# liangfu/dspnet

Hardware: AMD Instinct MI355X
Metric: training images/sec at 512x512 multitask (higher is better)
Workload: dtype f32; 1 GPU; resnet-50 multitask (det+depth+seg) 512x512, 8 det classes, 19 seg classes, N=6132 anchors, forward+backward+SGD; batch_per_gpu=32, global_batch=32, parallelism=dp1, f16x2_fallback_calls=0

## Files before the change

### dspnet_amd/csrc/conv.hip

```cpp
#include "dspn_common.h"
#include "bn_final_job.h"
#include "dspn_store.h"
#include "dspn_pieces.h"
#include "conv_geom.h"
#include <cstdlib>
#include "../../include/dspn_nn.h"

using dspn::st_t;
using dspn::kHalf;
using dspn::u32x4_t;

namespace {

using dspn::conv::f32x16;
using dspn::conv::bf16x8;
using dspn::pieces::bf16x4;
typedef __attribute__((address_space(3))) bf16x4 lds_bf16x4;

constexpr int kLdsRowH = kHalf ? 72 : 40;
__device__ __forceinline__ bf16x4 to_bf16x4(const float4 v) {
  bf16x4 r = {(__bf16)v.x, (__bf16)v.y, (__bf16)v.z, (__bf16)v.w};
  return r;
}

// ... 1227 lines not shown
  auto lo = [](int num, int den) { return num <= 0 ? 0 : (num + den - 1) / den; };
  const int ho_lo = lo(g.ph - r * g.dh, g.sh), wo_lo = lo(g.pw - q * g.dw, g.sw);
  const int ho_hi = min(g.Ho - 1, (g.H - 1 + g.ph - r * g.dh) / g.sh);
  const int wo_hi = min(g.Wo - 1, (g.W - 1 + g.pw - q * g.dw) / g.sw);
  const int rows_per = (g.Ho + g.chunks - 1) / g.chunks;
  const int h0 = max(ho_lo, chunk * rows_per), h1 = min(ho_hi, (chunk + 1) * rows_per - 1);
  const int KL = min(g.ldy, 256), PL = 256 / KL;
  const int kl = threadIdx.x % KL, pl = threadIdx.x / KL;
  for (int kb = 0; kb < g.ldy; kb += KL) {
    const int k = kb + kl;
    float s = 0.f;
    if (pl < PL && k < g.ldy && (g.H - 1 + g.ph - r * g.dh) >= 0 && (g.W - 1 + g.pw - q * g.dw) >= 0)
      for (int ho = h0; ho <= h1; ++ho)
        for (int wo = wo_lo + pl; wo <= wo_hi; wo += PL) s += p2[((long long)ho * g.Wo + wo) * g.ldy + k];
    sm[threadIdx.x] = s;
    __syncthreads();
    if (pl == 0 && k < g.ldy) {
      for (int j = 1; j < PL; ++j) s += sm[j * KL + kl];
      partial[((long long)tap * g.chunks + chunk) * g.ldy + k] = s;
    }
    __syncthreads();
  }
}
__global__ __launch_bounds__(1024) void sum_grad_final_kernel(const float *__restrict__ partial,
                                                              const float *__restrict__ w, float *__restrict__ out,
                                                              int taps, int chunks, int ldy, int Cout, int Cin) {
  __shared__ double sm[1024];
  double acc[8] = {0, 0, 0, 0, 0, 0, 0, 0};
  for (int i = threadIdx.x; i < taps * Cout; i += 1024) {
    const int tap = i / Cout, k = i - tap * Cout;
    double d = 0;
    for (int c = 0; c < chunks; ++c) d += partial[((long long)tap * chunks + c) * ldy + k];
    for (int c = 0; c < Cin; ++c) acc[c] += d * (double)w[((long long)k * taps + tap) * Cin + c];
  }
  for (int c = 0; c < Cin; ++c) {
    sm[threadIdx.x] = acc[c];
    __syncthreads();
    for (int st = 512; st >= 1; st >>= 1) {
      if ((int)threadIdx.x < st) sm[threadIdx.x] += sm[threadIdx.x + st];
      __syncthreads();
    }
    if (threadIdx.x == 0) out[c] = (float)sm[0];
    __syncthreads();
  }
}

__global__ void slab_reduce_kernel(const float4 *__restrict__ slab, float4 *__restrict__ dw,
                                   long long n4, int splits, int accumulate) {
  for (long long i = blockIdx.x * (long long)blockDim.x + threadIdx.x; i < n4;
       i += (long long)gridDim.x * blockDim.x) {
    float4 s = slab[i];
    int k = 1;
    for (; k + 16 <= splits; k += 16) {
      float4 v[16];
#pragma unroll
      for (int u = 0; u < 16; ++u) v[u] = slab[(long long)(k + u) * n4 + i];
#pragma unroll
      for (int u = 0; u < 16; ++u) { s.x += v[u].x; s.y += v[u].y; s.z += v[u].z; s.w += v[u].w; }
    }
    for (; k < splits; ++k) {
      const float4 v = slab[(long long)k * n4 + i];
      s.x += v.x; s.y += v.y; s.z += v.z; s.w += v.w;
    }
    if (accumulate) { const float4 v = dw[i]; s.x += v.x; s.y += v.y; s.z += v.z; s.w += v.w; }
    dw[i] = s;
  }
}

__global__ void weight_transpose_kernel(const float *__restrict__ w, st_t *__restrict__ wt, st_t *__restrict__ wh,
                                        int K, int T, int C, int Kp) {
  const long long total = (long long)C * T * Kp;
  for (long long i = blockIdx.x * (long long)blockDim.x + threadIdx.x; i < total;
       i += (long long)gridDim.x * blockDim.x) {
    const int k = (int)(i % Kp);
    const long long ct = i / Kp;
    const int t = (int)(ct % T), c = (int)(ct / T);
    const long long src = ((long long)k * T + t) * C + c;
    const float v = k < K ? w[src] : 0.f;
    wt[i] = (st_t)v;
    if (wh && k < K) wh[src] = (st_t)v;
  }
}

struct SlabDesc { const float4 *slab; float4 *dw; long long n4; int splits, accumulate; long long begin; };
__global__ void slab_reduce_batch_kernel(const SlabDesc *__restrict__ d, int n, long long total) {
  for (long long i = blockIdx.x * (long long)blockDim.x + threadIdx.x; i < total;
       i += (long long)gridDim.x * blockDim.x) {
    int lo = 0, hi = n - 1;
    while (lo < hi) {
      const int mid = (lo + hi + 1) >> 1;
      if (d[mid].begin <= i) lo = mid; else hi = mid - 1;
    }
    const SlabDesc e = d[lo];
    const long long j = i - e.begin;
    float4 s = e.slab[j];
    int k = 1;
    for (; k + 16 <= e.splits; k += 16) {
      float4 v[16];
#pragma unroll
      for (int u = 0; u < 16; ++u) v[u] = e.slab[(long long)(k + u) * e.n4 + j];
#pragma unroll
      for (int u = 0; u < 16; ++u) { s.x += v[u].x; s.y += v[u].y; s.z += v[u].z; s.w += v[u].w; }
    }
    for (; k < e.splits; ++k) {
      const float4 v = e.slab[(long long)k * e.n4 + j];
      s.x += v.x; s.y += v.y; s.z += v.z; s.w += v.w;
    }
    if (e.accumulate) { const float4 v = e.dw[j]; s.x += v.x; s.y += v.y; s.z += v.z; s.w += v.w; }
    e.dw[j] = s;
  }
}

struct WtDesc { const float *w; st_t *wt; int K, T, C, Kp; long long begin; st_t *wh; };
__global__ __launch_bounds__(256) void weight_transpose_batch_kernel(const WtDesc *__restrict__ d, int n) {
  __shared__ float sm[32][33];
  const long long tile_g = blockIdx.x;
  int lo = 0, hi = n - 1;
  while (lo < hi) {
    const int mid = (lo + hi + 1) >> 1;
    if (d[mid].begin <= tile_g) lo = mid; else hi = mid - 1;
  }
  const WtDesc e = d[lo];
  const long long tile = tile_g - e.begin;
  const int cblocks = (e.C + 31) >> 5;
  const int cb = (int)(tile % cblocks);
  const long long kt = tile / cblocks;
  const int t = (int)(kt % e.T), kb = (int)(kt / e.T);
  const int r = threadIdx.x >> 3, q = threadIdx.x & 7;
  {
    const int k = kb * 32 + r, c = cb * 32 + 4 * q;
    float4 v = make_float4(0.f, 0.f, 0.f, 0.f);
    if (k < e.K && c < e.C) {
      const long long src = ((long long)k * e.T + t) * e.C + c;
      v = *reinterpret_cast<const float4 *>(e.w + src);
      if (e.wh) st4(e.wh + src, v);
    }
    sm[r][4 * q] = v.x; sm[r][4 * q + 1] = v.y; sm[r][4 * q + 2] = v.z; sm[r][4 * q + 3] = v.w;
  }
  __syncthreads();
  const int cc = cb * 32 + r, kq = kb * 32 + 4 * q;
  if (cc < e.C && kq < e.Kp)
    st4(e.wt + ((long long)cc * e.T + t) * e.Kp + kq, make_float4(sm[4 * q][r], sm[4 * q + 1][r], sm[4 * q + 2][r], sm[4 * q + 3][r]));
}

struct WpDesc { const float *w; __bf16 *planes; __bf16 *planes_t; int K, T, C, cols_t; long long begin; const float *absmax; int npc, pad_; };
__device__ __forceinline__ void weight_planes_tile(const WpDesc &e, long long tile, __bf16 (*sm)[32][36]) {
  const int pb = e.npc * 32;
  const float scale = e.npc == 2 ? operand_scale(e.absmax) : 1.f;
  const int cblocks = (e.C + 31) >> 5;
  const int cb = (int)(tile % cblocks);
  const long long kt = tile / cblocks;
  const int t = (int)(kt % e.T), kb = (int)(kt / e.T);
  const int r = threadIdx.x >> 3, q = threadIdx.x & 7;
  const int k = kb * 32 + r, c = cb * 32 + 4 * q;
  float4 v = make_float4(0.f, 0.f, 0.f, 0.f);
  if (k < e.K && c < e.C) v = *reinterpret_cast<const float4 *>(e.w + ((long long)k * e.T + t) * e.C + c);
  bf16x4 p[3];
  if (e.npc == 2) { split2h(v, scale, p[0], p[1]); repair_inf(p[0], p[1]); p[2] = p[1]; }
  else split3(v, p[0], p[1], p[2]);
  if (e.planes && k < e.K && c < e.C) {
    __bf16 *d = e.planes + (((long long)k * e.T + t) * (e.C >> 5) + cb) * pb + 4 * q;
#pragma unroll
    for (int pc = 0; pc < 3; ++pc)
      if (pc < e.npc) *reinterpret_cast<bf16x4 *>(d + 32 * pc) = p[pc];
  }
  if (!e.planes_t) return;
#pragma unroll
  for (int pc = 0; pc < 3; ++pc)
#pragma unroll
    for (int i = 0; i < 4; ++i) sm[pc][4 * q + i][r] = p[pc][i];
  __syncthreads();
  const int cc = cb * 32 + r;
  if (cc < e.C && kb * 32 < e.cols_t) {
    __bf16 *d = e.planes_t + (((long long)cc * e.T + t) * (e.cols_t >> 5) + kb) * pb + 4 * q;
#pragma unroll
    for (int pc = 0; pc < 3; ++pc) {
      if (pc >= e.npc) break;
      bf16x4 o = {sm[pc][r][4 * q], sm[pc][r][4 * q + 1], sm[pc][r][4 * q + 2], sm[pc][r][4 * q + 3]};
      *reinterpret_cast<bf16x4 *>(d + 32 * pc) = o;
    }
  }
}
__global__ __launch_bounds__(256) void weight_planes_batch_kernel(const WpDesc *__restrict__ d, int n) {
  __shared__ __bf16 sm[3][32][36];
  const long long tile = blockIdx.x;
  int lo = 0, hi = n - 1;
  while (lo < hi) {
    const int mid = (lo + hi + 1) >> 1;
// ... 770 lines not shown
  } else
#endif
  if (BM == 32) DSPN_WGRAD_LAUNCH(1, 4, 1, 1)
  else if (BM == 64) DSPN_WGRAD_LAUNCH(2, 2, 1, 2)
  else if (BN == 64) DSPN_WGRAD_LAUNCH(2, 2, 2, 1)
  else DSPN_WGRAD_LAUNCH(4, 2, 1, 2)
#undef DSPN_WGRAD_LAUNCH
#undef DSPN_WGRAD_LAUNCH_
  int rc = dspn::check_launch("conv_wgrad");
  if (rc || !dw) return rc;
  const long long n4 = (long long)Cout * J / 4;
  const int blocks = (int)std::min<long long>((n4 + 255) / 256, 2048);
  hipLaunchKernelGGL(slab_reduce_kernel, dim3(blocks), dim3(256), 0, s,
                     reinterpret_cast<const float4 *>(slab), reinterpret_cast<float4 *>(dw), n4,
                     (int)splits, accumulate);
  return dspn::check_launch("conv_wgrad_reduce");
}

int DSPN_FN(dspn_conv2d_wgrad_bn)(const st_t *x, const float *in_scale, const float *in_shift, int in_relu,
                             const st_t *dy, float *dw, int N, int H, int W, int Cin,
                             int Cout, int ldy, int R, int S, int stride, int pad_h, int pad_w, int dil, int Ho,
                             int Wo, int accumulate, int math, const float *x_absmax, const float *dy_absmax,
                             void *workspace, size_t workspace_bytes, void *stream) {
  DSPN_REQUIRE(N > 0 && H > 0 && W > 0 && Cin > 0 && Ho > 0 && Wo > 0 && ldy > 0, "conv2d_wgrad: bad geometry");
  DSPN_REQUIRE((in_scale == nullptr) == (in_shift == nullptr), "conv2d_wgrad: in_scale and in_shift go together");
  const int math_vouch = math & DSPN_MATH_UNSCALED_OK;
  const int dy_planes = ((math & DSPN_MATH_DY_PLANES) ? 1 : 0) | ((math & DSPN_MATH_X_PLANES) ? 2 : 0);
  math &= ~(DSPN_MATH_UNSCALED_OK | DSPN_MATH_DY_PLANES | DSPN_MATH_X_PLANES);
  DSPN_REQUIRE(!(dy_planes & 1) || (!dspn::kHalf && math == DSPN_MATH_F32_F16X2 && ldy == Cout && Cout % 32 == 0 && dy_absmax),
               "conv2d_wgrad: DSPN_MATH_DY_PLANES needs DSPN_MATH_F32_F16X2, ldy == Cout, Cout %% 32 == 0 and the block the planes were cut by (dy_absmax)");
  DSPN_REQUIRE(!(dy_planes & 2) || (!dspn::kHalf && math == DSPN_MATH_F32_F16X2 && Cin % 32 == 0 && x_absmax && !in_scale),
               "conv2d_wgrad: DSPN_MATH_X_PLANES needs DSPN_MATH_F32_F16X2, Cin %% 32 == 0, no input affine and the block the planes were cut by (x_absmax)");
  DSPN_REQUIRE(math >= DSPN_MATH_FP32 && math <= DSPN_MATH_F32_F16X2, "conv2d_wgrad: math is one of DSPN_MATH_*");
  DSPN_REQUIRE(dspn::kHalf || math != DSPN_MATH_F32_F16X2 || math_vouch || (x_absmax && dy_absmax),
               "conv2d_wgrad: DSPN_MATH_F32_F16X2 needs the magnitude block of both operands (dspn_absmax_f32); a caller who knows that every |operand| < 65504 passes math | DSPN_MATH_UNSCALED_OK");
  const int nb = std::min(batch_chunk(N, (long long)sizeof(st_t) * H * W * Cin),
                          batch_chunk(N, (long long)sizeof(st_t) * Ho * Wo * ldy));
  for (int n0 = 0; n0 < N; n0 += nb) {
    const int n = std::min(nb, N - n0);
    const int rc = conv2d_wgrad_one(math, OpScales{dy_absmax, x_absmax, dy_planes}, x + (long long)n0 * H * W * Cin, InAffine{in_scale, in_shift, in_relu},
                                    dy + (long long)n0 * Ho * Wo * ldy, dw, n, H, W,
                                    Cin, Cout, ldy, R, S, stride, pad_h, pad_w, dil, Ho, Wo, accumulate || n0 > 0,
                                    workspace, workspace_bytes, stream);
    if (rc) return rc;
  }
  return 0;
}

#ifndef DSPN_HALF
int dspn_conv2d_wgrad_splits(int N, int Ho, int Wo, int Cin, int Cout, int R, int S, int stride) {
  const long long P = (long long)N * Ho * Wo;
  const int J = R * S * Cin;
  if (P <= 0 || J <= 0 || Cout <= 0) return 0;
  return wgrad_plan(P, Cout, J, R * S > 1 ? 4ll * P * Cin * std::min(stride, 2) * std::min(stride, 2) : 0).splits;
}
#endif

int DSPN_FN(dspn_conv2d_wgrad_slabs)(const st_t *x, const float *in_scale, const float *in_shift, int in_relu,
                                const st_t *dy, float *slabs, size_t slabs_bytes, int N, int H, int W, int Cin,
                                int Cout, int ldy, int R, int S, int stride, int pad_h, int pad_w, int dil, int Ho,
                                int Wo, int math, const float *x_absmax, const float *dy_absmax, void *stream) {
  DSPN_REQUIRE(N > 0 && H > 0 && W > 0 && Cin > 0 && Ho > 0 && Wo > 0 && ldy > 0, "conv2d_wgrad: bad geometry");
  DSPN_REQUIRE((in_scale == nullptr) == (in_shift == nullptr), "conv2d_wgrad: in_scale and in_shift go together");
  const int math_vouch = math & DSPN_MATH_UNSCALED_OK;
  const int dy_planes = ((math & DSPN_MATH_DY_PLANES) ? 1 : 0) | ((math & DSPN_MATH_X_PLANES) ? 2 : 0);
  math &= ~(DSPN_MATH_UNSCALED_OK | DSPN_MATH_DY_PLANES | DSPN_MATH_X_PLANES);
  DSPN_REQUIRE(!(dy_planes & 1) || (!dspn::kHalf && math == DSPN_MATH_F32_F16X2 && ldy == Cout && Cout % 32 == 0 && dy_absmax),
               "conv2d_wgrad: DSPN_MATH_DY_PLANES needs DSPN_MATH_F32_F16X2, ldy == Cout, Cout %% 32 == 0 and the block the planes were cut by (dy_absmax)");
  DSPN_REQUIRE(!(dy_planes & 2) || (!dspn::kHalf && math == DSPN_MATH_F32_F16X2 && Cin % 32 == 0 && x_absmax && !in_scale),
               "conv2d_wgrad: DSPN_MATH_X_PLANES needs DSPN_MATH_F32_F16X2, Cin %% 32 == 0, no input affine and the block the planes were cut by (x_absmax)");
  DSPN_REQUIRE(math >= DSPN_MATH_FP32 && math <= DSPN_MATH_F32_F16X2, "conv2d_wgrad: math is one of DSPN_MATH_*");
  DSPN_REQUIRE(dspn::kHalf || math != DSPN_MATH_F32_F16X2 || math_vouch || (x_absmax && dy_absmax),
               "conv2d_wgrad: DSPN_MATH_F32_F16X2 needs the magnitude block of both operands (dspn_absmax_f32); a caller who knows that every |operand| < 65504 passes math | DSPN_MATH_UNSCALED_OK");
  DSPN_REQUIRE(std::min(batch_chunk(N, (long long)sizeof(st_t) * H * W * Cin),
                        batch_chunk(N, (long long)sizeof(st_t) * Ho * Wo * ldy)) == N,
               "conv2d_wgrad_slabs: tensors of 2 GiB or more need dspn_conv2d_wgrad_f32");
  return conv2d_wgrad_one(math, OpScales{dy_absmax, x_absmax, dy_planes}, x, InAffine{in_scale, in_shift, in_relu}, dy, nullptr, N, H, W, Cin, Cout, ldy, R, S, stride,
                          pad_h, pad_w, dil, Ho, Wo, 0, slabs, slabs_bytes, stream);
}

#ifndef DSPN_HALF
int dspn_conv2d_slab_reduce_batch_f32(const void *table, int n, long long total4, void *stream) {
  DSPN_REQUIRE(table && n > 0 && total4 > 0, "slab_reduce_batch: bad argument");
  static_assert(sizeof(SlabDesc) == 40, "table row layout: 2 pointers, int64, 2 ints, int64");
  const int blocks = (int)std::min<long long>((total4 + 255) / 256, 16384);
  dspn::ProfScope prof(1, (hipStream_t)stream);
  hipLaunchKernelGGL(slab_reduce_batch_kernel, dim3(blocks), dim3(256), 0, (hipStream_t)stream,
                     static_cast<const SlabDesc *>(table), n, total4);
  return dspn::check_launch("slab_reduce_batch");
}

int dspn_conv2d_wgrad_f32(const float *x, const float *dy, float *dw, int N, int H, int W, int Cin,
                          int Cout, int ldy, int R, int S, int stride, int pad_h, int pad_w, int dil, int Ho,
                          int Wo, int accumulate, void *workspace, size_t workspace_bytes,
                          void *stream) {
  return dspn_conv2d_wgrad_bn_f32(x, nullptr, nullptr, 0, dy, dw, N, H, W, Cin, Cout, ldy, R, S, stride, pad_h, pad_w, dil,
                                  Ho, Wo, accumulate, DSPN_MATH_FP32, nullptr, nullptr, workspace, workspace_bytes, stream);
}

#endif

}
```

### dspnet_amd/csrc/nn.hip

```cpp
#include "dspn_common.h"
#include "bn_final_job.h"
#include "dspn_store.h"
#include "dspn_pieces.h"
#include "../../include/dspn_nn.h"

using dspn::st_t;
using dspn::A1Ptr;
using dspn::A4Ptr;
using dspn::CA1Ptr;
using dspn::CA4Ptr;

#pragma clang fp contract(fast)

namespace {

constexpr int kT = 256;
inline int slab_rows_for(long long rows) {
  const long long want = (rows + 1023) / 1024;
  return (int)std::min<long long>(512, std::max<long long>(32, (want + 7) / 8 * 8));
}

inline int grid_for(long long n, int per_block = kT, int cap = 8192) {
  long long b = (n + per_block - 1) / per_block;
  return (int)std::max<long long>(1, std::min<long long>(b, cap));
// ... 715 lines not shown
  const long long i = start + blockIdx.x * (long long)blockDim.x + threadIdx.x;
  if (i < n) o[i] = a[i] + b[i];
}
__global__ void relu_bwd_kernel(const CA1Ptr y, const CA1Ptr dy, const A1Ptr dx, long long n, int accumulate) {
  for (long long i = blockIdx.x * (long long)blockDim.x + threadIdx.x; i < n;
       i += (long long)gridDim.x * blockDim.x) {
    float v = y[i] > 0.f ? dy[i] : 0.f;
    if (accumulate) v += dx[i];
    dx[i] = v;
  }
}
#ifndef DSPN_HALF
__global__ void fill_kernel(float *p, float v, long long n) {
  for (long long i = blockIdx.x * (long long)blockDim.x + threadIdx.x; i < n;
       i += (long long)gridDim.x * blockDim.x)
    p[i] = v;
}
#endif

__global__ __launch_bounds__(kT) void colsum_partial_kernel(const CA1Ptr a,
                                                            long long rows, int C, int ld,
                                                            float *__restrict__ partial, int slab_rows) {
  __shared__ float sm[kT];
  const int CL = min(C, kT), RL = kT / CL;
  const int cl = threadIdx.x % CL, rl = threadIdx.x / CL;
  const long long r0 = (long long)blockIdx.x * slab_rows, r1 = min(rows, r0 + slab_rows);
  for (int cb = 0; cb < C; cb += CL) {
    const int c = cb + cl;
    float s = 0.f;
    if (rl < RL && c < C)
      for (long long r = r0 + rl; r < r1; r += RL) s += a[r * ld + c];
    sm[threadIdx.x] = s;
    __syncthreads();
    if (rl == 0 && c < C) {
      for (int k = 1; k < RL; ++k) s += sm[k * CL + cl];
      partial[(long long)blockIdx.x * C + c] = s;
    }
    __syncthreads();
  }
}
__global__ __launch_bounds__(kT) void relu_bwd_colsum_partial_kernel(const CA4Ptr y,
                                                                   const CA4Ptr dy,
                                                                   const A4Ptr dx, long long rows, int ld4,
                                                                   int CL, float *__restrict__ partial, int C,
                                                                   int slab_rows, unsigned *__restrict__ dx_absmax) {
  extern __shared__ __attribute__((aligned(16))) float4 sm4[];
  const int RL = kT / CL;
  const int cl = threadIdx.x % CL, rl = threadIdx.x / CL;
  const int c4 = blockIdx.y * CL + cl;
  const long long r0 = (long long)blockIdx.x * slab_rows, r1 = min(rows, r0 + slab_rows);
  float4 s = make_float4(0, 0, 0, 0);
  float mx = 0.f;
  if (rl < RL && c4 < ld4) {
#pragma unroll 4
    for (long long r = r0 + rl; r < r1; r += RL) {
      const float4 yv = y[r * ld4 + c4];
      float4 g = dy[r * ld4 + c4];
      g.x = yv.x > 0.f ? g.x : 0.f; g.y = yv.y > 0.f ? g.y : 0.f;
      g.z = yv.z > 0.f ? g.z : 0.f; g.w = yv.w > 0.f ? g.w : 0.f;
      dx[r * ld4 + c4] = g;
      s.x += g.x; s.y += g.y; s.z += g.z; s.w += g.w;
      mx = fmaxf(mx, fmaxf(fmaxf(fabsf(g.x), fabsf(g.y)), fmaxf(fabsf(g.z), fabsf(g.w))));
    }
  }
  if (dx_absmax) {
#pragma unroll
    for (int o = 32; o >= 1; o >>= 1) mx = fmaxf(mx, __shfl_xor(mx, o, 64));
    if ((threadIdx.x & 63) == 0 && mx > 0.f) atomicMax(dx_absmax + ((blockIdx.x * 4u + (threadIdx.x >> 6)) & 63u), __float_as_uint(mx));
  }
  sm4[threadIdx.x] = s;
  __syncthreads();
  if (rl == 0 && c4 < ld4) {
    for (int k = 1; k < RL; ++k) {
      const float4 a = sm4[k * CL + cl];
      s.x += a.x; s.y += a.y; s.z += a.z; s.w += a.w;
    }
    float *p = partial + (long long)blockIdx.x * C;
    const float v[4] = {s.x, s.y, s.z, s.w};
#pragma unroll
    for (int e = 0; e < 4; ++e)
      if (c4 * 4 + e < C) p[c4 * 4 + e] = v[e];
  }
}
__global__ __launch_bounds__(1024) void colsum_final_kernel(const float *partial, int nslabs, int C, float *out) {
  __shared__ double sm[64][17];
  const int cl = threadIdx.x & 15, sl = threadIdx.x >> 4;
  const int c = blockIdx.x * 16 + cl;
  double s = 0;
  if (c < C) {
#pragma unroll 8
    for (int k = sl; k < nslabs; k += 64) s += partial[(long long)k * C + c];
  }
  sm[sl][cl] = s;
  __syncthreads();
  if (sl == 0 && c < C) {
    for (int k = 1; k < 64; ++k) s += sm[k][cl];
    out[c] = (float)s;
  }
}

__global__ void nchw_to_nhwc_kernel(const float *__restrict__ src, const A1Ptr dst,
                                    int C, long long HW, long long total_pix, int Cp) {
  for (long long p = blockIdx.x * (long long)blockDim.x + threadIdx.x; p < total_pix;
       p += (long long)gridDim.x * blockDim.x) {
    const long long n = p / HW, hw = p - n * HW;
    for (int c = 0; c < Cp; ++c)
      dst[p * Cp + c] = c < C ? src[(n * C + c) * HW + hw] : 0.f;
  }
}
#ifndef DSPN_HALF
__global__ void nhwc_to_nchw_kernel(const float *__restrict__ src, float *__restrict__ dst,
                                    int C, long long HW, long long total, int Cp) {
  for (long long i = blockIdx.x * (long long)blockDim.x + threadIdx.x; i < total;
       i += (long long)gridDim.x * blockDim.x) {
    const long long hw = i % HW, nc = i / HW;
    const long long n = nc / C; const int c = (int)(nc - n * C);
    dst[i] = src[(n * HW + hw) * Cp + c];
  }
}
#endif
template <typename SRC, typename DST>
__global__ void copy_block_kernel(const SRC src, const DST dst,
                                  long long rows_per_sample, int C, long long sss, int lds, int soff,
                                  long long dss, int ldd, int doff, long long total, int accumulate) {
  for (long long i = blockIdx.x * (long long)blockDim.x + threadIdx.x; i < total;
       i += (long long)gridDim.x * blockDim.x) {
    const int c = (int)(i % C);
    const long long r = i / C;
    const long long s = r / rows_per_sample, rr = r - s * rows_per_sample;
    const float v = src[s * sss + rr * lds + soff + c];
    const long long di = s * dss + rr * ldd + doff + c;
    const float old = accumulate ? (float)dst[di] : 0.f;
    dst[di] = old + v;
  }
}
__global__ void copy_block_vec_kernel(const dspn::u32x4_t *__restrict__ src, dspn::u32x4_t *__restrict__ dst,
                                      long long rows_per_sample, int C, long long sss, int lds, int soff,
                                      long long dss, int ldd, int doff, long long total) {
  for (long long i = blockIdx.x * (long long)blockDim.x + threadIdx.x; i < total;
       i += (long long)gridDim.x * blockDim.x) {
    const int c = (int)(i % C);
    const long long r = i / C;
    const long long s = r / rows_per_sample, rr = r - s * rows_per_sample;
    dst[s * dss + rr * ldd + doff + c] = src[s * sss + rr * lds + soff + c];
  }
}
#ifndef DSPN_HALF
struct CopyDesc { const float *src; float *dst; long long rows_per_sample, sss, dss; int C, lds, soff, ldd, doff, accumulate; long long begin; };
static_assert(sizeof(CopyDesc) == 72, "copy_block_batch table row (dspnet_amd/functional.py copy_block_table)");
__global__ void copy_block_batch_kernel(const CopyDesc *__restrict__ d, int n, long long total) {
  for (long long i = blockIdx.x * (long long)blockDim.x + threadIdx.x; i < total;
       i += (long long)gridDim.x * blockDim.x) {
    int lo = 0, hi = n - 1;
    while (lo < hi) {
      const int mid = (lo + hi + 1) >> 1;
      if (d[mid].begin <= i) lo = mid; else hi = mid - 1;
    }
    const CopyDesc e = d[lo];
    const long long j = i - e.begin;
    const int c = (int)(j % e.C);
    const long long r = j / e.C;
    const long long sm = r / e.rows_per_sample, rr = r - sm * e.rows_per_sample;
    const float v = e.src[sm * e.sss + rr * e.lds + e.soff + c];
    const long long di = sm * e.dss + rr * e.ldd + e.doff + c;
    e.dst[di] = e.accumulate ? e.dst[di] + v : v;
  }
}
__global__ void transpose_bnc_kernel(const float *__restrict__ src, float *__restrict__ dst,
                                     int N, int C, long long total) {
  for (long long i = blockIdx.x * (long long)blockDim.x + threadIdx.x; i < total;
       i += (long long)gridDim.x * blockDim.x) {
    const int n = (int)(i % N);
    const long long bc = i / N;
    const int c = (int)(bc % C);
    const long long b = bc / C;
    dst[i] = src[(b * N + n) * C + c];
  }
}
#endif

// ... 961 lines not shown
                       reinterpret_cast<const float4 *>(shift), reinterpret_cast<const dspn::u32x4_t *>(dy),
                       reinterpret_cast<const float4 *>(coef), reinterpret_cast<dspn::u32x4_t *>(dx), n4 / 2, C / 8, relu,
                       accumulate, fixed8);
    return dspn::check_launch("bn_backward");
  }
#endif
  int fixed4 = 0, u4 = 0;
  const int grid4 = grid_fixed_channel(n4, C4, &fixed4, &u4);
  hipLaunchKernelGGL(u4 ? bn_bwd_apply_kernel<4> : bn_bwd_apply_kernel<1>, dim3(grid4), dim3(kT), 0, S_(stream),
                     CA4Ptr(x), reinterpret_cast<const float4 *>(scale),
                     reinterpret_cast<const float4 *>(shift), CA4Ptr(dy),
                     reinterpret_cast<const float4 *>(coef), A4Ptr(dx), n4, C4, relu,
                     accumulate, dspn::kHalf ? nullptr : reinterpret_cast<unsigned *>(dx_absmax), fixed4);
  return dspn::check_launch("bn_backward_from_sums");
}

int DSPN_FN(dspn_add)(const st_t *a, const st_t *b, st_t *out, long long n, void *stream) {
  DSPN_REQUIRE(a && b && out && n >= 0, "add: bad argument");
  const long long n4 = n / 4;
  if (n4 > 0)
    hipLaunchKernelGGL(add_kernel, dim3(grid_for(n4)), dim3(kT), 0, S_(stream),
                       CA4Ptr(a), CA4Ptr(b),
                       A4Ptr(out), n4);
  if (n4 * 4 < n)
    hipLaunchKernelGGL(add_tail_kernel, dim3(1), dim3(64), 0, S_(stream), CA1Ptr(a), CA1Ptr(b), A1Ptr(out), n4 * 4, n);
  return dspn::check_launch("add");
}

int DSPN_FN(dspn_relu_backward)(const st_t *y, const st_t *dy, st_t *dx, long long n, int accumulate,
                           void *stream) {
  DSPN_REQUIRE(y && dy && dx && n >= 0, "relu_backward: bad argument");
  if (n == 0) return 0;
  hipLaunchKernelGGL(relu_bwd_kernel, dim3(grid_for(n)), dim3(kT), 0, S_(stream), CA1Ptr(y), CA1Ptr(dy), A1Ptr(dx), n, accumulate);
  return dspn::check_launch("relu_backward");
}

int DSPN_FN(dspn_relu_backward_colsum)(const st_t *y, const st_t *dy, st_t *dx, long long rows, int C, int ld, float *out,
                                  float *dx_absmax, void *workspace, size_t workspace_bytes, void *stream) {
  DSPN_REQUIRE(!dx_absmax || !dspn::kHalf, "relu_backward_colsum: dx_absmax is for float tensors");
  DSPN_REQUIRE(y && dy && dx && out && workspace && rows > 0 && C > 0 && ld >= C && ld % 4 == 0,
               "relu_backward_colsum: bad argument");
  const int sr = colsum_slab_rows(rows);
  const int ns = (int)((rows + sr - 1) / sr);
  if (workspace_bytes < sizeof(float) * (size_t)ns * C)
    return dspn::fail(DSPN_ERR_WORKSPACE_, "relu_backward_colsum: workspace too small (dspn_colsum_workspace_bytes)");
  const int ld4 = ld / 4, CL = std::min(ld4, 64);
  float *partial = static_cast<float *>(workspace);
  hipLaunchKernelGGL(relu_bwd_colsum_partial_kernel, dim3(ns, (ld4 + CL - 1) / CL), dim3(kT), sizeof(float4) * kT,
                     S_(stream), CA4Ptr(y), CA4Ptr(dy),
                     A4Ptr(dx), rows, ld4, CL, partial, C, sr, reinterpret_cast<unsigned *>(dx_absmax));
  hipLaunchKernelGGL(colsum_final_kernel, dim3((C + 15) / 16), dim3(1024), 0, S_(stream), partial, ns, C, out);
  return dspn::check_launch("relu_backward_colsum");
}

#ifndef DSPN_HALF
int dspn_fill_f32(float *p, float v, long long n, void *stream) {
  DSPN_REQUIRE(p && n >= 0, "fill: bad argument");
  if (n == 0) return 0;
  hipLaunchKernelGGL(fill_kernel, dim3(grid_for(n)), dim3(kT), 0, S_(stream), p, v, n);
  return dspn::check_launch("fill");
}
#endif

#ifndef DSPN_HALF
size_t dspn_colsum_workspace_bytes(long long rows, int C) {
  if (rows <= 0 || C <= 0) return 0;
  const int sr = colsum_slab_rows(rows);
  return sizeof(float) * (size_t)((rows + sr - 1) / sr) * C;
}
#endif
int DSPN_FN(dspn_colsum)(const st_t *a, long long rows, int C, int ld, float *out, void *workspace,
                    size_t workspace_bytes, void *stream) {
  DSPN_REQUIRE(a && out && workspace && rows > 0 && C > 0 && ld >= C, "colsum: bad argument");
  const int sr = colsum_slab_rows(rows);
  const int ns = (int)((rows + sr - 1) / sr);
  if (workspace_bytes < sizeof(float) * (size_t)ns * C)
    return dspn::fail(DSPN_ERR_WORKSPACE_, "colsum: workspace too small");
  float *partial = static_cast<float *>(workspace);
  hipLaunchKernelGGL(colsum_partial_kernel, dim3(ns), dim3(kT), 0, S_(stream), CA1Ptr(a), rows, C, ld, partial, sr);
  hipLaunchKernelGGL(colsum_final_kernel, dim3((C + 15) / 16), dim3(1024), 0, S_(stream), partial, ns, C, out);
  return dspn::check_launch("colsum");
}

int DSPN_FN(dspn_nchw_to_nhwc)(const float *src, st_t *dst, int N, int C, int H, int W, int Cp, void *stream) {
  DSPN_REQUIRE(src && dst && N > 0 && C > 0 && H > 0 && W > 0 && Cp >= C, "nchw_to_nhwc: bad argument");
  const long long HW = (long long)H * W, total = HW * N;
  hipLaunchKernelGGL(nchw_to_nhwc_kernel, dim3(grid_for(total)), dim3(kT), 0, S_(stream), src, A1Ptr(dst), C, HW, total, Cp);
  return dspn::check_launch("nchw_to_nhwc");
}
#ifndef DSPN_HALF
int dspn_nhwc_to_nchw_f32(const float *src, float *dst, int N, int C, int H, int W, int Cp, void *stream) {
  DSPN_REQUIRE(src && dst && N > 0 && C > 0 && H > 0 && W > 0 && Cp >= C, "nhwc_to_nchw: bad argument");
  const long long HW = (long long)H * W, total = HW * N * C;
  hipLaunchKernelGGL(nhwc_to_nchw_kernel, dim3(grid_for(total)), dim3(kT), 0, S_(stream), src, dst, C, HW, total, Cp);
  return dspn::check_launch("nhwc_to_nchw");
}
#endif

int DSPN_FN(dspn_copy_block)(const st_t *src, st_t *dst, int samples, long long rows_per_sample, int C,
                        long long src_sample_stride, int lds, int soff, long long dst_sample_stride,
                        int ldd, int doff, int accumulate, void *stream) {
  DSPN_REQUIRE(src && dst && samples > 0 && rows_per_sample > 0 && C > 0, "copy_block: bad argument");
  const long long total = (long long)samples * rows_per_sample * C;
  constexpr int E = 16 / (int)sizeof(st_t);
  if (!accumulate && C % E == 0 && lds % E == 0 && ldd % E == 0 && soff % E == 0 && doff % E == 0 &&
      src_sample_stride % E == 0 && dst_sample_stride % E == 0 &&
      ((reinterpret_cast<uintptr_t>(src) | reinterpret_cast<uintptr_t>(dst)) & 15) == 0) {
    hipLaunchKernelGGL(copy_block_vec_kernel, dim3(grid_for(total / E)), dim3(kT), 0, S_(stream),
                       reinterpret_cast<const dspn::u32x4_t *>(src), reinterpret_cast<dspn::u32x4_t *>(dst), rows_per_sample,
                       C / E, src_sample_stride / E, lds / E, soff / E, dst_sample_stride / E, ldd / E, doff / E, total / E);
    return dspn::check_launch("copy_block");
  }
  hipLaunchKernelGGL((copy_block_kernel<CA1Ptr, A1Ptr>), dim3(grid_for(total)), dim3(kT), 0, S_(stream), CA1Ptr(src),
                     A1Ptr(dst), rows_per_sample, C, src_sample_stride, lds, soff, dst_sample_stride, ldd, doff,
                     total, accumulate);
  return dspn::check_launch("copy_block");
}
#ifndef DSPN_HALF
int dspn_copy_block_batch_f32(const void *table, int n, long long total, void *stream) {
  DSPN_REQUIRE(table && n > 0 && total > 0, "copy_block_batch: bad argument");
  hipLaunchKernelGGL(copy_block_batch_kernel, dim3(grid_for(total)), dim3(kT), 0, S_(stream),
                     static_cast<const CopyDesc *>(table), n, total);
  return dspn::check_launch("copy_block_batch");
}
#endif
#ifdef DSPN_HALF
int dspn_copy_block_bf16_f32(const st_t *src, float *dst, int samples, long long rows_per_sample, int C,
                             long long src_sample_stride, int lds, int soff, long long dst_sample_stride,
                             int ldd, int doff, int accumulate, void *stream) {
  DSPN_REQUIRE(src && dst && samples > 0 && rows_per_sample > 0 && C > 0, "copy_block: bad argument");
  const long long total = (long long)samples * rows_per_sample * C;
  hipLaunchKernelGGL((copy_block_kernel<CA1Ptr, float *>), dim3(grid_for(total)), dim3(kT), 0, S_(stream), CA1Ptr(src),
                     dst, rows_per_sample, C, src_sample_stride, lds, soff, dst_sample_stride, ldd, doff, total,
                     accumulate);
  return dspn::check_launch("copy_block");
}
int dspn_copy_block_f32_bf16(const float *src, st_t *dst, int samples, long long rows_per_sample, int C,
                             long long src_sample_stride, int lds, int soff, long long dst_sample_stride,
                             int ldd, int doff, int accumulate, void *stream) {
  DSPN_REQUIRE(src && dst && samples > 0 && rows_per_sample > 0 && C > 0, "copy_block: bad argument");
  const long long total = (long long)samples * rows_per_sample * C;
  hipLaunchKernelGGL((copy_block_kernel<const float *, A1Ptr>), dim3(grid_for(total)), dim3(kT), 0, S_(stream), src,
                     A1Ptr(dst), rows_per_sample, C, src_sample_stride, lds, soff, dst_sample_stride, ldd, doff, total,
                     accumulate);
  return dspn::check_launch("copy_block");
}
#endif

#ifndef DSPN_HALF
int dspn_transpose_bnc_f32(const float *src, float *dst, int B, int N, int C, void *stream) {
  DSPN_REQUIRE(src && dst && B > 0 && N > 0 && C > 0, "transpose_bnc: bad argument");
  const long long total = (long long)B * N * C;
  hipLaunchKernelGGL(transpose_bnc_kernel, dim3(grid_for(total)), dim3(kT), 0, S_(stream), src, dst, N, C, total);
  return dspn::check_launch("transpose_bnc");
}
#endif

int DSPN_FN(dspn_tap_sum)(const st_t *z, const float *bias, st_t *y, int N, int H, int W, int Cout, int ldy,
                     int ldz, int R, int S, int pad_h, int pad_w, void *stream) {
  DSPN_REQUIRE(z && y && N > 0 && H > 0 && W > 0 && Cout > 0 && ldy >= Cout && ldz >= Cout * R * S,
               "tap_sum: bad argument");
  const long long total = (long long)N * H * W * ldy;
  hipLaunchKernelGGL(tap_sum_kernel_, dim3(grid_for(total, kT, 65535)), dim3(kT), 0, S_(stream), CA1Ptr(z), bias, A1Ptr(y), H, W,
                     Cout, ldy, ldz, R, S, pad_h, pad_w, total);
  return dspn::check_launch("tap_sum");
}
// ... 261 lines not shown
```

### dspnet_amd/engine.py

```python
import math
import os
import re

import numpy as np
import torch

from . import functional as fn, graph_plan


FUSE_BATCHNORM = True
COMMUTE_RESIZE_CONV = True
MATERIALISE_MULTITAP_INPUT_BF16 = os.environ.get("DSPN_MAT3X3", "1") != "0"


_SHARED_STREAMS = {}


def shared_stream(device, kind, priority=0):
    key = (str(device), kind)
    ent = _SHARED_STREAMS.get(key)
    if ent is None:
        ent = _SHARED_STREAMS[key] = (torch.cuda.Stream(device=device, priority=priority), priority)
    assert ent[1] == priority, "shared stream %r of %s was created with priority %d, asked for %d" % (kind, device, ent[1], priority)
    return ent[0]
# ... 79 lines not shown
            self._wg.before_write(self.grad)
            fn.add(self.grad, buf, out=self.grad)


class Param:
    def __init__(self, name, shape, init, wd_mult=1.0):
        self.name, self.shape, self.init, self.wd_mult = name, tuple(shape), init, wd_mult
        self.fixed, self.lr_mult = False, 1.0
        self.data = self.grad = None
        self.offset = 0
        self.logical = None
        self.kind = "vec"

    @property
    def size(self):
        return int(np.prod(self.shape))


class Wiring:

    def __init__(self, outputs):
        self.outputs = outputs
        self.reads = []
        self.params = []

    def record(self, node):
        made = {id(t) for t in self.outputs}
        for k, v in vars(node).items():
            for t in (v.values() if isinstance(v, dict) else v if isinstance(v, (list, tuple)) else (v,)):
                if isinstance(t, Tensor) and id(t) not in made:
                    self.reads.append((k, t))
                elif isinstance(t, Param):
                    self.params.append(t)


class Node:

    def __init_subclass__(cls, **kw):
        super().__init_subclass__(**kw)
        init = cls.__dict__.get("__init__")
        if init is None:
            return

        def wrapped(self, g, *args, __init=init, **kwargs):
            if "wiring" in self.__dict__:
                return __init(self, g, *args, **kwargs)
            start = len(g.all_tensors)
            self.wiring = None
            __init(self, g, *args, **kwargs)
            self.wiring = Wiring(g.all_tensors[start:])
        wrapped.__wrapped__ = init
        cls.__init__ = wrapped

    def forward(self):
        raise NotImplementedError

    def backward(self):
        pass


class Graph:
    def __init__(self, device):
        self.device = device
        self.nodes = []
        self.params = {}
        self.param_order = []
        self.bn_names = []
        self.bn_nodes = {}
        self.bn_momentum, self.bn_global = 0.9, False
        self.bn_track = False
        self.tensors = {}
        self.all_tensors = []
        self.pre_forward = []
        self.wgrad_side_allowed = True
        self.wg = WgradSide(device)
        self._bn_chain = None
        self.side_segment = None
        self.side_pending = False
        self.side_bwd = None
        self.side_fwd_events, self.side_fwd_waits = {}, {}
        self.side_plan = None
        self.slab_tables = {}
        self.wt_table = None
        self.wt_batched = False
        self.arena = self.grad_arena = self.mom_arena = None
        self.half_operands = False
        self.math = fn.get_conv_math()
        self.wp_table = None
        self._nscal = 0
        self.scalars = None
        self.am_table = None
        self._am_x = {}
        self._am_wanted = set()
        self._am_done = set()
        self._am_bwd_slots, self._am_bwd_ran = set(), False
        self._am_table_slots = set()
        self.scalars_min = None
        self.guard = dict(enabled=os.environ.get("DSPN_RANGE_GUARD", "1") != "0", have_stats=False, risk=frozenset(),
                          calls=0, calls_total=0, at_risk_slots=0)
        self.wmin_table = None
        self.fixed_names, self.freeze_re, self.freezing = frozenset(), None, False
        self.wt_frozen = self.wp_frozen = self.am_frozen = self.wmin_frozen = None
        self.frozen_stale = False
        self._nscal_step = 0

    def set_freeze(self, fixed_param_names=None, freeze_pattern=None):
        assert not self.nodes, "set_freeze() before the graph is built"
        self.fixed_names = frozenset(fixed_param_names or ())
        self.freeze_re = re.compile(freeze_pattern) if freeze_pattern else None
        self.freezing = bool(self.fixed_names) or self.freeze_re is not None

    def is_fixed(self, name):
        return name in self.fixed_names or (self.freeze_re is not None and self.freeze_re.match(name) is not None)

    @property
    def fixed_param_names(self):
        return sorted(p.name for p in self.param_order if p.fixed)

    def tensor(self, shape, name, requires_grad=True, data=None, virtual=False, dtype=None):
        t = Tensor(self, shape, name, requires_grad, data=data, virtual=virtual, dtype=dtype)
        assert name not in self.tensors, "duplicate tensor name " + name
        self.tensors[name] = t
        self.all_tensors.append(t)
        return t

    def param(self, name, shape, init):
        assert name not in self.params, name
        p = Param(name, shape, init)
        p.fixed = self.freezing and self.is_fixed(name)
        self.params[name] = p
        self.param_order.append(p)
        return p

    def add(self, node):
        self.nodes.append(node)
        w = node.wiring
        w.record(node)
        if self.freezing and all(p.fixed for p in w.params) and not any(t.requires_grad for _, t in w.reads):
            for t in w.outputs:
                t.requires_grad = False
        return node

    def new_scalar(self, backward=False):
        self._nscal += 1
        if backward:
            self._am_bwd_slots.add(self._nscal - 1)
        return self._nscal - 1

    def scalar(self, i):
        return None if (i is None or self.scalars is None) else self.scalars[i * fn.ABSMAX_SLOTS:(i + 1) * fn.ABSMAX_SLOTS]

    def want_magnitude(self, t):
        while t is not None:
            if t.am_slot is not None:
                self._am_wanted.add(t.am_slot)
            t = t.alias_of

    def magnitude(self, slot, tensor, src=None):
        if slot is None or self.scalars is None or tensor.dtype != torch.float32:
            return None
        if src is not None and src.am_slot is not None and src.am_slot in self._am_done:
            return self.scalar(src.am_slot)
        out = self.scalar(slot)
        if slot not in self._am_done:
            fn.absmax(tensor, out=out)
            self._am_done.add(slot)
# ... 27 lines not shown
        gd["calls"] = 0
        capturing = self.device.type == "cuda" and torch.cuda.is_current_stream_capturing()
        if capturing:
            gd["wmin_now"] = True
            return
        gd["count"] = gd.get("count", 0) + 1
        gd["wmin_now"] = blocking or gd["count"] % self.GUARD_PERIOD == self.GUARD_PERIOD - 1 or not gd["have_stats"]
        if not gd["enabled"] or self.scalars is None or not gd["have_stats"]:
            return
        if not blocking and gd["count"] % self.GUARD_PERIOD != 0:
            return
        both = self._guard_fetch(blocking)
        if both is not None:
            self._guard_decide(both)

    def _guard_fetch(self, blocking):
        gd = self.guard
        if blocking:
            gd["queue"] = []
            return self._spans_device().cpu().numpy()
        pool = gd.setdefault("pinned", [torch.empty((2, self.scalars_min.numel()), dtype=torch.float32, pin_memory=True)
                                        for _ in range(3)])
        host = pool[gd.get("pin_i", 0) % 3]
        gd["pin_i"] = gd.get("pin_i", 0) + 1
        host.copy_(self._spans_device(), non_blocking=True)
        ev = torch.cuda.Event()
        ev.record()
        gd.setdefault("queue", []).append((host, ev))
        if len(gd["queue"]) < 2:
            return None
        host, ev = gd["queue"].pop(0)
        ev.synchronize()
        return host.numpy()

    def _guard_decide(self, both):
        gd = self.guard
        mx, mn = both[0], both[1]
        ok = np.isfinite(mn) & (mn > 0) & (mx > 0)
        wide = np.zeros(mx.shape, bool)
        wide[ok] = np.log2(mx[ok] / mn[ok]) > self.GUARD_BITS
        gd["at_risk_slots"] = int(wide.sum())
        risk = set()
        if wide.any():
            for n in self.nodes:
                if isinstance(n, Conv) and n.am_x is not None and not n.tap_expand:
                    if wide[n.am_x] or wide[n.am_w] or wide[n.am_dy]:
                        risk.add(id(n))
        if risk == gd["risk"]:
            return False
        gd["risk"] = frozenset(risk)
        for n in self.nodes:
            if isinstance(n, Conv):
                n.guard_fb = id(n) in risk
        return True

    def guard_poll(self, blocking=False):
        gd = self.guard
        if not gd["enabled"] or self.scalars is None or not gd["have_stats"]:
            return False
        both = self._guard_fetch(blocking)
        return both is not None and self._guard_decide(both)

    def guard_report(self):
        return len(self.guard["risk"]), self.guard["calls"], self.guard["at_risk_slots"]

    def finalize(self, seed=0):
        graph_plan.plan(self)
        self._wt_pairs_nodes = [n for n in self.nodes if isinstance(n, Conv) and (n.wt is not None or n.wh is not None)]
        off = 0
        for p in self.param_order:
            p.offset = off
            off += (p.size + 3) // 4 * 4
        self.arena = torch.zeros(off, dtype=torch.float32, device=self.device)
        self.grad_arena = torch.zeros_like(self.arena)
        self.mom_arena = torch.zeros_like(self.arena)
        rng = np.random.Generator(np.random.PCG64(seed))
        host = np.zeros(off, np.float32)
        for p in self.param_order:
            host[p.offset:p.offset + p.size] = np.asarray(p.init(rng, p.shape), np.float32).reshape(-1)
        self.arena.copy_(torch.from_numpy(host))
        for p in self.param_order:
            p.data = self.arena[p.offset:p.offset + p.size].view(p.shape)
            p.grad = self.grad_arena[p.offset:p.offset + p.size].view(p.shape)
        if self._wt_pairs_nodes and self.device.type == "cuda":
            for n in self._wt_pairs_nodes:
                if n.wt is None:
                    n.wt = fn.zeros(n.w.shape[3], n.w.shape[1], n.w.shape[2], n.out.shape[3], device=self.device,
                                    dtype=n.wh.dtype)
            pairs = [n for n in self._wt_pairs_nodes if n.wtp is None or n.wh is not None]
            for frozen in (False, True):
                rows = [(n.w.data, n.wt, n.wh) for n in pairs if n.w.fixed == frozen]
                if rows:
                    tab = fn.weight_transpose_table(rows, self.device)
                    setattr(self, "wt_frozen" if frozen else "wt_table", tab)
                    self.half_operands = tab[3]
        if self.device.type == "cuda":
            wnodes = [n for n in self.nodes if getattr(n, "am_w", None) is not None and getattr(n, "w", None) is not None]
            self._nscal_step = self._nscal
            for n in wnodes:
                if n.w.fixed:
                    n.am_w = self.new_scalar()
                    if isinstance(n, Deconv4x4s2):
                        n.am = (n.am[0], n.am_w, n.am[2])
            if self.math == "f16x2" and self._nscal:
                self.scalars = torch.zeros(self._nscal * fn.ABSMAX_SLOTS, dtype=torch.float32, device=self.device)
                self.scalars_min = torch.full((self._nscal,), float("inf"), dtype=torch.float32, device=self.device)
                self._am_table_slots = {n.am_w for n in wnodes}
                for frozen in (False, True):
                    sel = [n for n in wnodes if n.w.fixed == frozen]
                    if not sel:
                        continue
                    am = fn.absmax_table([(n.w.data, self.scalar(n.am_w)) for n in sel], self.device)
                    wmin = (fn.absmin_rows_table([(n.w.data.view(n.w.shape[0], -1), self.scalars_min[n.am_w:n.am_w + 1])
                                                  for n in sel], self.device) if self.guard["enabled"] else None)
                    if frozen:
                        self.am_frozen, self.wmin_frozen = am, wmin
                    else:
                        self.am_table, self.wmin_table = am, wmin
            convs = [n for n in self.nodes if isinstance(n, Conv) and (n.wp is not None or n.wtp is not None)]
            for frozen in (False, True):
                planes = [(n.w.data, n.wp, n.wtp) + ((self.scalar(n.am_w),) if self.math == "f16x2" else ())
                          for n in convs if n.w.fixed == frozen]
                if planes:
                    setattr(self, "wp_frozen" if frozen else "wp_table", fn.weight_planes_table(planes, self.device))
            self.frozen_stale = any(t is not None for t in (self.wt_frozen, self.wp_frozen, self.am_frozen))
        if self.device.type == "cuda":
            for n in self.nodes:
                if isinstance(n, Conv):
                    n.alloc_slabs()
        return self

    def flush_slabs(self, key="all", convs=None, beside=False):
        nodes, table = self._slab_table(key, convs if convs is not None else self.nodes)
        wg = self.wg
        beside = beside and wg.last is not None
        if not beside:
            self.wgrad_beside_join()
        if not nodes:
            return
        ran = [n for n in nodes if n.slabs_fresh]
        if ran:
            args = table if len(ran) == len(nodes) else self._slab_table(frozenset(map(id, ran)), ran)[1]
            if beside:
                main, side = torch.cuda.current_stream(self.device), wg.stream
                ev = wg.event()
                ev.record(main)
                side.wait_event(ev)
                with torch.cuda.stream(side):
                    fn.slab_reduce_batch(*args)
                    done = wg.event()
                    done.record(side)
                wg.last = done
            else:
                fn.slab_reduce_batch(*args)
        for n in nodes:
            n.slabs_fresh = False

    def _slab_table(self, key, convs):
        if key not in self.slab_tables:
            nodes = [n for n in convs if isinstance(n, Conv) and n.slabs is not None]
            table = fn.slab_reduce_table([(n.slabs, n.w.grad, False) for n in nodes], self.device) if nodes else None
            self.slab_tables[key] = (nodes, table)
        return self.slab_tables[key]

    def load_params(self, values):
        self.frozen_stale = self.frozen_stale or any(self.params[k].fixed for k in values)
        for k, v in values.items():
            self.params[k].data.copy_(torch.from_numpy(np.ascontiguousarray(v, np.float32)).view(self.params[k].shape))

    def _node_tensors(self, n):
        seen, out = set(), []

        def take(t):
            while t is not None and id(t) not in seen:
                seen.add(id(t))
                out.append(t)
                if t.affine_src is not None:
                    take(t.affine_src[0])
                t = t.alias_of

        for t in [t for _, t in n.wiring.reads] + n.wiring.outputs:
            take(t)
        return out

    def forward(self):
        self.wt_batched = False
        if self.half_operands:
            fn.weight_transpose_batch(*self.wt_table)
            self.wt_batched = True
        if self.scalars is not None:
            self._update_guard(blocking=self.guard.pop("decide_now", False))
            self.scalars[:self._nscal_step * fn.ABSMAX_SLOTS].zero_()
            self.scalars_min[:self._nscal_step].fill_(float("inf"))
            if self.wmin_table is not None and self.guard.get("wmin_now", True):
                fn.absmin_rows_batch(*self.wmin_table)
            self._am_done = set()
            self._am_bwd_ran = False
            if self.am_table is not None:
                fn.absmax_batch(*self.am_table)
                self._am_done |= self._am_table_slots
        self.refresh_frozen()
        if self.wp_table is not None:
            fn.weight_planes_batch(*self.wp_table)
        for f in self.pre_forward:
            f()
        seg = self.side_segment
        if seg is None:
            for n in self.nodes:
                n.forward()
            self.guard["have_stats"] = True
            return
        first, last, side, ready, done = seg
        self.join_side()
        for i, n in enumerate(self.nodes):
            if i < first or i > last:
                for src in self.side_fwd_waits.get(i, ()):
                    torch.cuda.current_stream(self.device).wait_event(self.side_fwd_events[src])
                n.forward()
                continue
            if i == first:
                ready.record(torch.cuda.current_stream(self.device))
                side.wait_event(ready)
            with torch.cuda.stream(side), fn.workspace_lane(1):
                n.forward()
                if i in self.side_fwd_events:
                    self.side_fwd_events[i].record(side)
                if i == last:
                    done.record(side)
                    self.side_pending = True
        self.guard["have_stats"] = True

    def refresh_frozen(self):
        if not self.frozen_stale:
            return
        self.frozen_stale = False
        if self.wt_frozen is not None:
            fn.weight_transpose_batch(*self.wt_frozen)
        if self.scalars is not None:
            self.scalars[self._nscal_step * fn.ABSMAX_SLOTS:].zero_()
            self.scalars_min[self._nscal_step:].fill_(float("inf"))
            if self.wmin_frozen is not None:
                fn.absmin_rows_batch(*self.wmin_frozen)
            if self.am_frozen is not None:
                fn.absmax_batch(*self.am_frozen)
        if self.wp_frozen is not None:
            fn.weight_planes_batch(*self.wp_frozen)

    def set_side_segment(self, first, last):
        assert 0 <= first <= last < len(self.nodes)
        self.side_plan = dict(first=first, last=last, bwd=None)
        if self.device.type == "cuda":
            self.side_segment = (first, last, shared_stream(self.device, "branch", -1), torch.cuda.Event(), torch.cuda.Event())

    def set_side_backward(self, side_nodes, lo, hi, fork_after):
        assert self.side_plan is not None and all(lo <= i <= hi for i in side_nodes) and fork_after > hi
        self.side_plan["bwd"] = dict(side=frozenset(side_nodes), lo=lo, hi=hi, fork_after=fork_after)
        if self.side_segment is not None:
            self.side_bwd = dict(side=frozenset(side_nodes), lo=lo, hi=hi, fork_after=fork_after, fork_ev=torch.cuda.Event(),
                                 prog_ev=torch.cuda.Event(), forked=False, dirty=False, active=True)

    def backward_node(self, idx):
        sb, n = self.side_bwd, self.nodes[idx]
        if sb is None or not sb["active"]:
            n.backward()
            return
        if idx in sb["side"]:
            side = self.side_segment[2]
            if not sb["forked"]:
                side.wait_event(sb["fork_ev"])
# ... 337 lines not shown
            args, kw, _ = self._pending
            self._pending = None
            fn.bn_backward_from_sums(*args, phase=2, **kw)
            return
        if not self.out._gw:
            return
        am = None
        dgam = None if self.gamma is None else (fn.NO_OUTPUT if self.gamma.fixed else self.gamma.grad)
        dbet = fn.NO_OUTPUT if self.beta.fixed else self.beta.grad
        if self.x.requires_grad:
            dx, acc = self.x.grad_target()
            prod, g = self.x.producer, self._g
            if (isinstance(prod, Conv) and prod.am_dy is not None and g.scalars is not None and dx.dtype == torch.float32
                    and self.completes_x_grad):
                am = g.scalar(prod.am_dy)
                g._am_done.add(prod.am_dy)
        else:
            dx, acc = fn.NO_OUTPUT, False
        if self.pool_grad is not None:
            argmax, dyp, k, s, p = self.pool_grad
            self.pool_grad = None
            if not acc:
                fn.bn_backward_maxpool(self.x.data, self.scale, self.shift, dyp, argmax, k, s, p, self.mean, self.rstd,
                                       None if self.gamma is None else self.gamma.data, relu=self.relu, dx=dx,
                                       dgamma=dgam, dbeta=dbet, dx_absmax=am)
                return
            fn.maxpool_backward_argmax(argmax, dyp, self.out.shape, k, s, p, dx=self.out.own_grad())
            self.out.grad = self.out.own_grad()
        if (self.bwd_sums_ready and self.dx_planes and am is not None and not acc and self._x_ext_valid()
                and not getattr(prod, "guard_fb", False)):
            self.bwd_sums_ready = False
            self._from_sums(beside, (self.x.data, self.scale, self.shift, self.out.grad, self.mean, self.rstd,
                                     None if self.gamma is None else self.gamma.data, self.bwd_sums[0], self.bwd_sums[1]),
                            dict(relu=self.relu, dx=dx, dgamma=dgam, dbeta=dbet, accumulate=False, dx_absmax=am,
                                 dy_absmax=self._g.scalar(self.am_dyin), x_chan_minmax=self.x_ext, dx_planes=True,
                                 dx_absmin=g.scalars_min[prod.am_dy:prod.am_dy + 1] if g.guard["enabled"] else None))
            self.x.grad_planes = True
            return
        if self.bwd_sums_ready:
            self.bwd_sums_ready = False
            self._from_sums(beside, (self.x.data, self.scale, self.shift, self.out.grad, self.mean, self.rstd,
                                     None if self.gamma is None else self.gamma.data, self.bwd_sums[0], self.bwd_sums[1]),
                            dict(relu=self.relu, dx=dx, dgamma=dgam, dbeta=dbet, accumulate=acc, dx_absmax=am))
            return
        assert not beside, "finalize_beside() without the data gradient's sums"
        fn.bn_backward(self.x.data, self.scale, self.shift, self.out.grad, self.mean, self.rstd,
                       None if self.gamma is None else self.gamma.data, relu=self.relu, dx=dx, dgamma=dgam, dbeta=dbet,
                       accumulate=acc, dx_absmax=am)


WGRAD_SIDE = int(os.environ.get("DSPN_WGRAD_SIDE", "1"))
WGRAD_SIDE_MIN_US = float(os.environ.get("DSPN_WGRAD_SIDE_MIN_US", "30"))

FINALIZE_BESIDE = os.environ.get("DSPN_FINALIZE_BESIDE", "1") != "0"

FUSE_CONV_MAGNITUDES = os.environ.get("DSPN_CONV_MAGNITUDES", "1") != "0"


def xa_unavailable(conv):
    return conv.out.data is None or conv.out.data.shape[-1] % 4 != 0


class Conv(Node):

    def __init__(self, g, x, name, num_filter, kernel, stride=1, pad=0, dilate=1, no_bias=True, relu=False,
                 init="xavier", cin_logical=None, cout_phys=None, input_sum_grad=None, residual=None, out_name=None,
                 tap_expand=False):
        N, H, W, Cin = x.shape
        kh, kw = fn._hw(kernel)
        ph, pw = fn._hw(pad)
        self.x, self.stride, self.pad, self.dil, self.relu = x, stride, (ph, pw), dilate, relu
        self.x_raw, self.in_affine = x, None
        if x.affine_src is not None:
            raw, sc, sh, arelu = x.affine_src
            self.x_raw, self.in_affine = raw, (sc, sh, arelu)
            assert not tap_expand
            x.bn_node.conv_consumers.append(self)
        elif x.bn_node is not None and not tap_expand:
            x.bn_node.mat_consumers.append(self)
        self.cout = num_filter
        self.input_sum_grad = input_sum_grad
        cin_meta = cin_logical if cin_logical is not None else (x.channels or Cin)
        cin_logical = Cin if cin_logical is None else cin_logical
        self.w = g.param(name + "_weight", (num_filter, kh, kw, Cin), conv_weight_init(init, cin_logical))
        self.b = None if no_bias else g.param(name + "_bias", (num_filter,), init_zeros)
        self.w.logical, self.w.kind = (num_filter, cin_meta, kh, kw), "conv"
        if self.b is not None:
            self.b.logical = (num_filter,)
        Ho, Wo = fn.conv_out_size(H, kh, stride, ph, dilate), fn.conv_out_size(W, kw, stride, pw, dilate)
        ldc = fn.padc(num_filter) if cout_phys is None else cout_phys
        self.out = g.tensor((N, Ho, Wo, ldc), out_name or (name + "_out"))
        self.out.channels = num_filter
        self.out.producer = self
        self.slabs, self.slabs_fresh = None, False
        self.out_stats = None
        self.out_minmax = None
        self._g = g
        self.residual = residual
        assert residual is None or residual.shape == self.out.shape
        half = self.out.dtype == torch.bfloat16
        self.wt_shape = (Cin, kh, kw, ldc)
        planes_t = g.device.type == "cuda" and x.requires_grad and fn.needs_planes(self.out.dtype, ldc, g.math)
        self.wt = None if (not x.requires_grad or planes_t) else fn.zeros(Cin, kh, kw, ldc, device=g.device, dtype=self.out.dtype)
        self.wh = fn.zeros(num_filter, kh, kw, Cin, device=g.device, dtype=torch.bfloat16) if half else None
        self.math = g.math
        self.am_x = self.am_dy = self.am_w = None
        if g.math == "f16x2" and self.out.dtype == torch.float32:
            key = (id(self.x_raw), None if self.in_affine is None else id(self.in_affine[0]))
            if key not in g._am_x:
                g._am_x[key] = g.new_scalar()
            self.am_x, self.am_dy, self.am_w = g._am_x[key], g.new_scalar(backward=True), g.new_scalar()
        self.am_out = g.new_scalar() if (self.am_x is not None and not tap_expand) else None
        if self.am_out is not None:
            self.out.am_slot = self.am_out
        if self.am_x is not None and self.in_affine is None:
            g.want_magnitude(self.x_raw)
        self.x_planes_bn = None
        self.bn_bwd_node = None
        self._wg_worth = None
        self.guard_fb = False
        self.wp = self.wtp = None
        if g.device.type == "cuda":
            npc = fn.plane_pieces(g.math)
            if fn.needs_planes(self.out.dtype, Cin, g.math):
                self.wp = fn.zeros(num_filter, kh * kw, Cin // 32, npc, 32, device=g.device, dtype=torch.bfloat16)
            if x.requires_grad and fn.needs_planes(self.out.dtype, ldc, g.math):
                self.wtp = fn.zeros(Cin, kh * kw, ldc // 32, npc, 32, device=g.device, dtype=torch.bfloat16)
        self.tap_expand = bool(tap_expand) and kh * kw > 1
        if self.tap_expand:
            assert stride == 1 and dilate == 1 and not relu and residual is None
            assert (Ho, Wo) == (H, W), "tap expansion needs a 'same' convolution"
            self.z = fn.act_zeros(N, H, W, fn.padc(num_filter * kh * kw), device=g.device)
        self.flops_fwd = 2.0 * cin_logical * num_filter * kh * kw * Ho * Wo * N
        self.flops_bwd = self.flops_fwd * (2 if x.requires_grad else 1)

    def alloc_slabs(self):
        if self.w.fixed:
            return
        cout, kh, kw, cin = self.w.shape
        wshape = (cout * kh * kw, 1, 1, cin) if self.tap_expand else self.w.shape
        xs = self.x.shape
        splits = fn.conv2d_wgrad_splits(xs, self.z.shape if self.tap_expand else self.out.shape, wshape,
                                        1 if self.tap_expand else self.stride)
        if splits > 0 and self.w.data.numel() % 4 == 0:
            self.slabs = fn.zeros(splits, self.w.data.numel(), device=self._g.device)

    def wop(self):
        return self.w.data if self.wh is None else self.wh

    def enable_out_stats(self):
        if self.tap_expand or self.out.shape[3] != self.cout or self.cout % 4 != 0:
            return None
        if self.out_stats is None:
            rows = self.out.shape[0] * self.out.shape[1] * self.out.shape[2]
            tiles, tile_rows = fn.conv_stats_layout(rows, self.cout)
            if tiles == 0:
                return None
            self.out_stats = (fn.zeros(tiles, 2, self.cout, device=self._g.device), tiles, tile_rows)
            if self.math == "f16x2" and self.out.dtype == torch.float32:
                self.out_minmax = fn.zeros(tiles, 2, self.cout, device=self._g.device)
        return self.out_stats

    def _magnitudes(self, which):
        g = self._g
        if self.am_x is None or g.scalars is None:
            return None
        if which == "x" and self.am_x not in g._am_done:
            src = self.x_raw
            while src.alias_of is not None:
                src = src.alias_of
            prod = src.producer
            table = getattr(prod, "out_minmax", None) if getattr(prod, "out", None) is src else None
            if table is not None:
                fn.absmax(table.view(-1, table.shape[-1]), self.in_affine, out=g.scalar(self.am_x))
            elif src.am_slot is not None and src.am_slot in g._am_done:
                if self.in_affine is None:
                    return g.scalar(src.am_slot)
                fn.absmax_affine_bound(self.in_affine[0], self.in_affine[1], g.scalar(src.am_slot), g.scalar(self.am_x))
            else:
                fn.absmax(self.x_raw.data, self.in_affine, out=g.scalar(self.am_x))
            g._am_done.add(self.am_x)
        return g.scalar({"x": self.am_x, "dy": self.am_dy, "w": self.am_w}[which])

    def forward(self):
        xa, wa = self._magnitudes("x"), self._magnitudes("w")
        if self.tap_expand:
            cout, kh, kw, cin = self.w.shape
            fn.conv2d_forward(self.x.data, self.wop().view(cout * kh * kw, 1, 1, cin), None, 1, 0, 1, out=self.z,
                              w_planes=self.wp, math=self.math,
                              x_absmax=xa, w_absmax=wa)
            fn.tap_sum(self.z, None if self.b is None else self.b.data, cout, kh, kw, self.pad, out=self.out.data)
            return
        if self.guard_fb:
            return self._forward_fallback()
        xp = self._x_planes()
        oa = self._out_magnitude()
        fn.conv2d_forward(self.x_raw.data if xp is None else xp, self.wop(), None if self.b is None else self.b.data, self.stride,
                          self.pad, self.dil, relu=self.relu, out=self.out.data,
                          residual=None if self.residual is None else self.residual.data,
                          in_affine=self.in_affine if xp is None else None,
                          out_stats=None if self.out_stats is None else self.out_stats[0], w_planes=self.wp,
                          math=self.math, x_absmax=xa, w_absmax=wa, out_minmax=self.out_minmax, x_planes=xp is not None,
                          out_absmax=oa)
        if oa is not None:
            self._g._am_done.add(self.am_out)

    def _out_magnitude(self):
        g = self._g
        if (not FUSE_CONV_MAGNITUDES or self.am_out is None or g.scalars is None or self.out_stats is not None
                or self.am_out not in g._am_wanted or xa_unavailable(self)):
            return None
        return g.scalar(self.am_out)

    def _x_planes(self):
        bn = self.x_planes_bn
        if self.guard_fb:
            return None
        return bn.planes if (bn is not None and bn.planes_ready and self.am_x in self._g._am_done) else None

    def _w3(self, transposed):
        cols = self.wt_shape[3] if transposed else self.w.shape[3]
        if cols % 32 != 0:
            return None
        return fn.weight_planes(self.w.data, transposed=transposed, cols=cols, math="bf16x3")

    def _forward_fallback(self):
        fn.conv2d_forward(self.x_raw.data, self.wop(), None if self.b is None else self.b.data, self.stride, self.pad, self.dil,
                          relu=self.relu, out=self.out.data, residual=None if self.residual is None else self.residual.data,
                          in_affine=self.in_affine, out_stats=None if self.out_stats is None else self.out_stats[0],
                          w_planes=self._w3(False), math="bf16x3")
        if self.out_minmax is not None:
            fn.tile_minmax(self.out.data, self.out_stats[2], self.out_minmax)
        oa = self._out_magnitude()
        if oa is not None:
            fn.absmax(self.out.data, out=oa)
            self._g._am_done.add(self.am_out)
        self._g.guard["calls"] += 1
        self._g.guard["calls_total"] += 1

    def backward(self):
        if not self.out._gw:
            return
        dy = self.out.grad
        planes = self.out.grad_planes
        if self.relu and self.b is not None:
            dya0 = None
            if (FUSE_CONV_MAGNITUDES and self.am_dy is not None and self._g.scalars is not None
                    and self.am_dy not in self._g._am_done and dy.dtype == torch.float32):
                dya0 = self._g.scalar(self.am_dy)
            fn.relu_backward_colsum(self.out.data, dy, self.cout, dx=dy, out=self.b.grad, dx_absmax=dya0)
            if dya0 is not None:
                self._g._am_done.add(self.am_dy)
        elif self.relu:
            fn.relu_backward(self.out.data, dy, dx=dy)
        if self.residual is not None and self.residual.requires_grad:
            self.residual.give_grad(dy)
        if self.b is not None and not self.relu and not self.b.fixed:
            fn.colsum(dy, self.cout, out=self.b.grad)
        xa, dya, wa = self._magnitudes("x"), self._magnitudes("dy"), self._magnitudes("w")
        if dya is not None and self.am_dy not in self._g._am_done:
            fn.absmax(dy, out=dya)
            self._g._am_done.add(self.am_dy)
        bn = self.bn_bwd_node if self.x.requires_grad else None
        isg = self.input_sum_grad if (self.input_sum_grad is not None and not self.input_sum_grad.fixed) else None
        if self.w.fixed:
            if isg is not None:
                fn.conv2d_input_sum_grad(dy, self.w.data, self.x.shape, self.stride, self.pad, self.dil, out=isg.grad)
            if self.x.requires_grad:
                self._data_gradient(dy, planes, dya, wa)
            return
        early = (bn is not None and FINALIZE_BESIDE and not self.guard_fb and self._g.device.type == "cuda"
                 and bn.pool_grad is None)
        if (WGRAD_SIDE and self._g.wgrad_side_allowed and self._g.device.type == "cuda" and (bn is not None or self._g.batchnorm_chain()) and self._wgrad_worth_a_stream()
                and self._g.wgrad_beside(self, dy, planes, xa, dya)):
            early = False
            if isg is not None:
                fn.conv2d_input_sum_grad(dy, self.w.data, self.x.shape, self.stride, self.pad, self.dil, out=isg.grad)
            if self.x.requires_grad:
                self._data_gradient(dy, planes, dya, wa)
            return
        if early:
            self._data_gradient(dy, planes, dya, wa)
            bn.finalize_beside()
        self._weight_gradient(dy, planes, xa, dya)
        if isg is not None:
            fn.conv2d_input_sum_grad(dy, self.w.data, self.x.shape, self.stride, self.pad, self.dil, out=isg.grad)
        if self.x.requires_grad and not early:
            self._data_gradient(dy, planes, dya, wa)

    def _wgrad_worth_a_stream(self):
        w = self._wg_worth
        if w is None:
            P = float(np.prod(self.out.shape[:-1]))
            cout, kh, kw, cin = self.w.shape
            esz = 4.0 if self.out.dtype == torch.float32 else 2.0
            est = max(2.0 * P * cout * kh * kw * cin / 2.5e14, esz * (P * cout + float(np.prod(self.x.shape))) / 4e12)
            w = self._wg_worth = est * 1e6 >= WGRAD_SIDE_MIN_US
        return w

    def _weight_gradient(self, dy, planes, xa, dya):
        if self.tap_expand:
            cout, kh, kw, cin = self.w.shape
            fn.tap_spread(dy, cout, kh, kw, self.pad, out=self.z)
            if self.slabs is not None:
                fn.conv2d_wgrad_slabs(self.x.data, self.z, (cout * kh * kw, 1, 1, cin), self.slabs, 1, 0, 1, math=self.math,
                                      x_absmax=xa)
            else:
                fn.conv2d_wgrad(self.x.data, self.z, (cout * kh * kw, 1, 1, cin), 1, 0, 1,
                                out=self.w.grad.view(cout * kh * kw, 1, 1, cin), math=self.math, x_absmax=xa)
        elif self.guard_fb:
            assert not planes, "a convolution on the guard's fallback got its gradient as piece planes"
            if self.slabs is not None:
                fn.conv2d_wgrad_slabs(self.x_raw.data, dy, self.w.shape, self.slabs, self.stride, self.pad, self.dil,
                                      in_affine=self.in_affine, math="bf16x3")
            else:
                fn.conv2d_wgrad(self.x_raw.data, dy, self.w.shape, self.stride, self.pad, self.dil, out=self.w.grad,
                                in_affine=self.in_affine, math="bf16x3")
            self._g.guard["calls"] += 1
            self._g.guard["calls_total"] += 1
        elif self.slabs is not None:
            xp = self._x_planes()
            fn.conv2d_wgrad_slabs(self.x_raw.data if xp is None else xp, dy, self.w.shape, self.slabs, self.stride, self.pad,
                                  self.dil, in_affine=self.in_affine if xp is None else None, math=self.math, x_absmax=xa,
                                  dy_absmax=dya, dy_planes=planes, x_planes=xp is not None)
        else:
            xp = self._x_planes()
            fn.conv2d_wgrad(self.x_raw.data if xp is None else xp, dy, self.w.shape, self.stride, self.pad, self.dil,
                            out=self.w.grad, in_affine=self.in_affine if xp is None else None, math=self.math, x_absmax=xa,
                            dy_absmax=dya, dy_planes=planes, x_planes=xp is not None)
        self.slabs_fresh = self.slabs is not None

    def _data_gradient(self, dy, planes, dya, wa):
        g = self._g
        if self.wtp is not None and (g.wp_frozen if self.w.fixed else g.wp_table) is None:
            fn.weight_planes(self.w.data, transposed=True, cols=self.wtp.shape[2] * 32, out=self.wtp, math=self.math,
                             w_absmax=wa)
        elif self.wtp is None and not (g.wt_frozen is not None if self.w.fixed else g.wt_batched):
            fn.weight_transpose(self.w.data, out=self.wt, copy=self.wh)
        dx, acc = self.x.grad_target()
        bn = self.bn_bwd_node
        bn_bwd, bn_dya = None, None
        if bn is not None:
            bn_bwd = (bn.x.data, bn.scale, bn.shift, bn.mean, bn.rstd, bn.relu, bn.bwd_sums[0])
            bn.bwd_sums_ready = True
            if bn.dx_planes:
                bn_dya = self._g.scalar(bn.am_dyin)
        if self.guard_fb:
            w3 = self._w3(True)
            fn.conv2d_dgrad(dy, self.wt if w3 is None else None, self.x.shape, self.stride, self.pad, self.dil, out=dx,
                            accumulate=acc, bn_bwd=bn_bwd, wt_planes=w3, math="bf16x3", wt_shape=self.wt_shape)
            if bn_dya is not None:
                fn.absmax(dx, out=bn_dya)
            self._g.guard["calls"] += 1
            self._g.guard["calls_total"] += 1
            return
        fn.conv2d_dgrad(dy, self.wt, self.x.shape, self.stride, self.pad, self.dil, out=dx, accumulate=acc,
                        bn_bwd=bn_bwd, wt_planes=self.wtp, math=self.math, dy_absmax=dya, w_absmax=wa,
                        bn_dy_absmax=bn_dya, dy_planes=planes, wt_shape=self.wt_shape)


class BilinearConcatConv(Node):

    def __init__(self, g, inputs, name, num_filter, kernel, pad, target_hw, theta, init="maxdim"):
        N = inputs[0].shape[0]
        kh, kw = fn._hw(kernel)
        self.pad = fn._hw(pad)
        assert (kh - 1) // 2 == self.pad[0] and (kw - 1) // 2 == self.pad[1], "needs a 'same' convolution"
        Ht, Wt = target_hw
        self.inputs = inputs
        self.theta = theta
        self.offsets = np.cumsum([0] + [t.shape[3] for t in inputs]).tolist()
        Cin = self.offsets[-1]
        self.cout, self.kh, self.kw = num_filter, kh, kw
        self.w = g.param(name + "_weight", (num_filter, kh, kw, Cin), conv_weight_init(init, Cin))
        self.w.logical, self.w.kind = (num_filter, Cin, kh, kw), "conv"
        T = num_filter * kh * kw
        Tp = fn.padc(T)
        self.T = T
        half = fn.ACT_DTYPE == torch.bfloat16
        self.z = fn.act_zeros(N, Ht, Wt, Tp, device=g.device)
        self.zc, self.wc, self.wct, self.dwc, self.wch, self.wcp = [], [], [], [], [], []
        self.math = g.math
        self._g = g
        f16 = g.math == "f16x2"
        self.am = [(g.new_scalar(), g.new_scalar(), g.new_scalar(backward=True)) if f16 else (None, None, None) for _ in inputs]
        self.am_w = g.new_scalar() if f16 else None
        for t in inputs:
            self.zc.append(fn.act_zeros(N, t.shape[1], t.shape[2], Tp, device=g.device))
            self.wc.append(fn.zeros(T, 1, 1, t.shape[3], device=g.device))
            self.wct.append(fn.act_zeros(t.shape[3], 1, 1, Tp, device=g.device))
            self.wch.append(fn.act_zeros(T, 1, 1, t.shape[3], device=g.device) if half else None)
            self.dwc.append(fn.zeros(T, 1, 1, t.shape[3], device=g.device))
            self.wcp.append(fn.zeros(T, 1, t.shape[3] // 32, fn.plane_pieces(g.math), 32, device=g.device, dtype=torch.bfloat16)
                            if g.device.type == "cuda" and fn.needs_planes(self.zc[-1].dtype, t.shape[3], g.math) else None)
        self.sources = None
        self.tpart = None
        self.out = g.tensor((N, Ht, Wt, fn.padc(num_filter)), name + "_out")
        self.out.channels = num_filter
        self.flops_fwd = sum(2.0 * t.shape[3] * T * t.shape[1] * t.shape[2] * N for t in inputs)
        self.flops_bwd = self.flops_fwd + sum(2.0 * t.shape[3] * T * t.shape[1] * t.shape[2] * N
                                              for t in inputs if t.requires_grad)
        self.flops_direct = 2.0 * Cin * T * Ht * Wt * N

    def _gather_weights(self):
        w2d = self.w.data
        Cin = self.offsets[-1]
        for c, t in enumerate(self.inputs):
            fn.copy_block(w2d, self.wc[c], 1, self.T, t.shape[3], 0, Cin, self.offsets[c], 0, t.shape[3], 0)

    def forward(self):
        self._gather_weights()
        for c, t in enumerate(self.inputs):
            if self.wch[c] is not None:
                fn.weight_transpose(self.wc[c], out=self.wct[c], copy=self.wch[c])
            xa, wa = self._g.magnitude(self.am[c][0], t.data, src=t), self._g.scalar(self.am_w)
            if self.wcp[c] is not None:
                fn.weight_planes(self.wc[c], out=self.wcp[c], math=self.math, w_absmax=wa)
            fn.conv2d_forward(t.data, self.wc[c] if self.wch[c] is None else self.wch[c], None, 1, 0, 1, out=self.zc[c],
                              w_planes=self.wcp[c], math=self.math, x_absmax=xa, w_absmax=wa)
        if self.sources is None:
            self.sources = fn.SamplerSources([(z, 0) for z in self.zc])
        fn.affine_sampler_forward(self.sources, self.theta.data, self.z)
        fn.tap_sum(self.z, None, self.cout, self.kh, self.kw, self.pad, out=self.out.data)

    def backward(self):
        if not self.out._gw:
            return
        fn.tap_spread(self.out.grad, self.cout, self.kh, self.kw, self.pad, out=self.z)
        if self.tpart is None:
            rows = [fn.affine_sampler_theta_rows(z.shape, self.z.shape[1], z.dtype) for z in self.zc]
            self.tpart = torch.zeros(sum(rows), 6, dtype=torch.float64, device=self.z.device)
            self.tpart_off = np.cumsum([0] + rows).tolist()
        Cin = self.offsets[-1]
        for c, t in enumerate(self.inputs):
            dza = self._g.scalar(self.am[c][2])
            if dza is not None and self.zc[c].dtype == torch.float32:
                self._g._am_done.add(self.am[c][2])
            dz = fn.affine_sampler_backward_data_theta(self.z, self.theta.data, self.zc[c], 0,
                                                       self.tpart[self.tpart_off[c]:self.tpart_off[c + 1]], dx=self.zc[c],
                                                       dx_absmax=dza)
            xa, wa = self._g.magnitude(self.am[c][0], t.data, src=t), self._g.scalar(self.am_w)
# ... 226 lines not shown
```

### dspnet_amd/functional.py

```python
import ctypes
import os

import numpy as np
import torch

from . import _lib
from ._lib import check

_c = ctypes
_vp = _c.c_void_p
_i = _c.c_int
_ll = _c.c_longlong
_f = _c.c_float
_sz = _c.c_size_t

_lib.register({
    "dspn_conv2d_split_workspace_bytes": (_sz, [_ll, _i]),
    "dspn_conv2d_forward_f32": (_i, [_vp, _vp, _vp, _vp, _vp, _i, _i, _i, _i, _i, _i, _i, _i, _i, _i, _i, _i, _i,
                                     _ll, _i, _i, _i, _vp, _sz, _vp]),
    "dspn_conv2d_forward_bn_f32": (_i, [_vp, _vp, _vp, _i, _vp, _vp, _vp, _vp, _vp, _i, _i, _i, _i, _i, _i, _i, _i, _i, _i, _i, _i,
                                        _i, _ll, _i, _i, _i, _vp, _sz, _vp, _i, _vp, _vp, _vp, _sz, _vp]),
    "dspn_absmax_f32": (_i, [_vp, _ll, _i, _vp, _vp, _i, _vp, _vp]),
    "dspn_absmax_batch_f32": (_i, [_vp, _i, _ll, _vp]),
    "dspn_conv2d_weight_planes_f32": (_i, [_vp, _vp, _vp, _i, _i, _i, _i, _i, _vp, _vp]),
    "dspn_conv2d_weight_planes_tiles": (_ll, [_i, _i, _i, _i, _i]),
    "dspn_conv2d_weight_planes_batch_f32": (_i, [_vp, _i, _ll, _vp]),
    "dspn_conv2d_stats_layout": (_i, [_ll, _i, _c.POINTER(_c.c_int)]),
    "dspn_bn_stats_from_tiles_f32": (_i, [_vp, _i, _i, _ll, _i, _f, _vp, _vp, _vp, _vp, _vp, _vp, _vp, _i, _vp, _vp, _vp, _vp, _sz, _vp]),
    "dspn_bn_tiles_workspace_bytes": (_sz, [_i, _i]),
    "dspn_conv2d_wgrad_bn_f32": (_i, [_vp, _vp, _vp, _i, _vp, _vp, _i, _i, _i, _i, _i, _i, _i, _i, _i, _i, _i, _i, _i, _i,
                                      _i, _i, _vp, _vp, _vp, _sz, _vp]),
    "dspn_conv2d_wgrad_splits": (_i, [_i, _i, _i, _i, _i, _i, _i, _i]),
    "dspn_conv2d_wgrad_slabs_f32": (_i, [_vp, _vp, _vp, _i, _vp, _vp, _sz, _i, _i, _i, _i, _i, _i, _i, _i, _i, _i, _i, _i,
                                         _i, _i, _i, _vp, _vp, _vp]),
    "dspn_conv2d_slab_reduce_batch_f32": (_i, [_vp, _i, _ll, _vp]),
    "dspn_conv2d_weight_transpose_batch_f32": (_i, [_vp, _i, _ll, _vp]),
    "dspn_conv2d_weight_transpose_tiles": (_ll, [_i, _i, _i, _i]),
    "dspn_conv2d_weight_transpose_f32": (_i, [_vp, _vp, _i, _i, _i, _i, _vp]),
    "dspn_conv2d_dgrad_f32": (_i, [_vp, _vp, _vp, _i, _i, _i, _i, _i, _i, _i, _i, _i, _i, _i, _i, _i, _i, _i, _vp,
                                   _sz, _vp]),
    "dspn_conv2d_dgrad_bn_tiles": (_i, [_i, _i, _i, _i, _i]),
    "dspn_conv2d_dgrad_bn_f32": (_i, [_vp, _vp, _vp, _vp, _i, _i, _i, _i, _i, _i, _i, _i, _i, _i, _i, _i, _i, _i, _i,
                                      _vp, _vp, _vp, _vp, _vp, _i, _vp, _sz, _vp, _i, _vp, _vp, _vp, _sz, _vp]),
    "dspn_bn_backward_from_sums_f32": (_i, [_vp, _vp, _vp, _vp, _vp, _vp, _vp, _vp, _i, _vp, _vp, _vp, _ll, _i, _i, _i,
                                            _vp, _vp, _vp, _vp, _i, _vp, _sz, _vp]),
    "dspn_bn_discard_parked": (_i, [_vp]),
    "dspn_absmin_rows_batch_f32": (_i, [_vp, _i, _ll, _vp]),
    "dspn_tile_minmax_f32": (_i, [_vp, _ll, _i, _i, _vp, _vp]),
    "dspn_conv2d_input_sum_grad_workspace_bytes": (_sz, [_i, _i, _i, _i, _i]),
    "dspn_conv2d_input_sum_grad_f32": (_i, [_vp, _vp, _vp, _i, _i, _i, _i, _i, _i, _i, _i, _i, _i, _i, _i, _i, _i,
                                            _vp, _sz, _vp]),
    "dspn_conv2d_wgrad_workspace_bytes": (_sz, [_i, _i, _i, _i, _i, _i, _i]),
    "dspn_conv2d_wgrad_f32": (_i, [_vp, _vp, _vp, _i, _i, _i, _i, _i, _i, _i, _i, _i, _i, _i, _i, _i, _i, _i,
                                   _vp, _sz, _vp]),
    "dspn_bn_workspace_bytes": (_sz, [_ll, _i]),
    "dspn_bn_stats_f32": (_i, [_vp, _ll, _i, _f, _vp, _vp, _vp, _vp, _vp, _vp, _vp, _sz, _vp]),
    "dspn_bn_apply_f32": (_i, [_vp, _vp, _vp, _vp, _ll, _i, _i, _vp, _vp]),
    "dspn_bn_apply_planes_f32": (_i, [_vp, _vp, _vp, _vp, _ll, _i, _i, _vp, _vp]),
    "dspn_absmax_affine_bound_f32": (_i, [_vp, _vp, _i, _vp, _vp, _vp]),
    "dspn_bn_backward_f32": (_i, [_vp, _vp, _vp, _vp, _vp, _vp, _vp, _vp, _vp, _vp, _ll, _i, _i, _i, _vp, _vp, _sz,
                                  _vp]),
    "dspn_add_f32": (_i, [_vp, _vp, _vp, _ll, _vp]),
    "dspn_relu_backward_f32": (_i, [_vp, _vp, _vp, _ll, _i, _vp]),
    "dspn_fill_f32": (_i, [_vp, _f, _ll, _vp]),
    "dspn_relu_backward_colsum_f32": (_i, [_vp, _vp, _vp, _ll, _i, _i, _vp, _vp, _vp, _sz, _vp]),
    "dspn_colsum_workspace_bytes": (_sz, [_ll, _i]),
    "dspn_colsum_f32": (_i, [_vp, _ll, _i, _i, _vp, _vp, _sz, _vp]),
    "dspn_nchw_to_nhwc_f32": (_i, [_vp, _vp, _i, _i, _i, _i, _i, _vp]),
    "dspn_nhwc_to_nchw_f32": (_i, [_vp, _vp, _i, _i, _i, _i, _i, _vp]),
    "dspn_copy_block_f32": (_i, [_vp, _vp, _i, _ll, _i, _ll, _i, _i, _ll, _i, _i, _i, _vp]),
    "dspn_copy_block_batch_f32": (_i, [_vp, _i, _ll, _vp]),
    "dspn_transpose_bnc_f32": (_i, [_vp, _vp, _i, _i, _i, _vp]),
    "dspn_avgpool2d_forward_f32": (_i, [_vp, _vp, _i, _i, _i, _i, _i, _i, _i, _i, _i, _vp]),
    "dspn_avgpool2d_backward_f32": (_i, [_vp, _vp, _i, _i, _i, _i, _i, _i, _i, _i, _i, _i, _vp]),
    "dspn_bilinear_backward_workspace_bytes": (_sz, [_i, _i, _i, _i]),
    "dspn_bilinear_backward_ws_f32": (_i, [_vp, _vp, _i, _i, _i, _i, _i, _i, _i, _i, _vp, _sz, _vp]),
    "dspn_seg_counts_f32": (_i, [_vp, _vp, _ll, _i, _i, _vp, _vp]),
    "dspn_seg_upsample_argmax_f32": (_i, [_vp, _vp, _i, _i, _i, _i, _i, _i, _i, _vp]),
    "dspn_tap_sum_f32": (_i, [_vp, _vp, _vp, _i, _i, _i, _i, _i, _i, _i, _i, _i, _i, _vp]),
    "dspn_tap_spread_f32": (_i, [_vp, _vp, _i, _i, _i, _i, _i, _i, _i, _i, _i, _i, _vp]),
    "dspn_maxpool_forward_f32": (_i, [_vp, _vp, _vp, _i, _i, _i, _i, _i, _i, _i, _i, _i, _vp]),
    "dspn_maxpool_forward_bn_f32": (_i, [_vp, _vp, _vp, _i, _vp, _vp, _i, _i, _i, _i, _i, _i, _i, _i, _i, _vp, _vp]),
    "dspn_maxpool_backward_argmax_f32": (_i, [_vp, _vp, _vp, _i, _i, _i, _i, _i, _i, _i, _i, _i, _vp]),
    "dspn_bn_backward_maxpool_f32": (_i, [_vp, _vp, _vp, _vp, _vp, _i, _i, _i, _i, _i, _i, _i, _i, _i, _vp, _vp, _vp, _vp, _vp,
                                          _vp, _i, _vp, _vp, _sz, _vp]),
    "dspn_maxpool_backward_f32": (_i, [_vp, _vp, _vp, _vp, _i, _i, _i, _i, _i, _i, _i, _i, _i, _vp]),
    "dspn_avgpool_forward_f32": (_i, [_vp, _vp, _i, _i, _i, _i, _i, _i, _i, _vp]),
    "dspn_avgpool_backward_f32": (_i, [_vp, _vp, _i, _i, _i, _i, _i, _i, _i, _i, _vp]),
    "dspn_bilinear_forward_f32": (_i, [_vp, _vp, _i, _i, _i, _i, _i, _i, _i, _i, _vp]),
    "dspn_bilinear_forward_acc_f32": (_i, [_vp, _vp, _i, _i, _i, _i, _i, _i, _i, _i, _vp]),
    "dspn_bilinear_backward_f32": (_i, [_vp, _vp, _i, _i, _i, _i, _i, _i, _i, _i, _vp]),
    "dspn_affine_sampler_forward_f32": (_i, [_vp, _vp, _vp, _vp, _vp, _i, _vp, _vp, _i, _i, _i, _i, _vp]),
    "dspn_affine_sampler_backward_data_f32": (_i, [_vp, _vp, _vp, _i, _i, _i, _i, _i, _i, _i, _i, _i, _vp]),
    "dspn_affine_sampler_theta_workspace_bytes": (_sz, [_i, _i, _i]),
    "dspn_affine_sampler_backward_theta_f32": (_i, [_vp, _vp, _vp, _vp, _vp, _i, _vp, _vp, _i, _i, _i, _i, _vp, _i,
                                                    _vp, _sz, _vp]),
    "dspn_affine_sampler_backward_data_theta_f32": (_i, [_vp, _vp, _vp, _vp, _i, _i, _i, _i, _i, _i, _i, _i, _i, _vp, _sz, _vp,
                                                         _vp, _sz, _vp]),
    "dspn_affine_sampler_theta_rows": (_ll, [_i, _i, _i, _i]),
    "dspn_affine_sampler_backward_workspace_bytes": (_sz, [_i, _i, _i, _i, _i]),
    "dspn_affine_sampler_theta_reduce_workspace_bytes": (_sz, [_ll]),
    "dspn_affine_sampler_theta_reduce": (_i, [_vp, _ll, _vp, _i, _vp, _sz, _vp]),
    "dspn_softmax_output_f32": (_i, [_vp, _vp, _vp, _vp, _ll, _i, _i, _f, _f, _vp, _vp]),
    "dspn_count_f32": (_i, [_vp, _ll, _i, _f, _vp, _vp]),
    "dspn_smooth_l1_forward_f32": (_i, [_vp, _vp, _vp, _vp, _ll, _vp]),
    "dspn_smooth_l1_backward_f32": (_i, [_vp, _vp, _vp, _vp, _ll, _f, _vp, _vp]),
    "dspn_cross_entropy_sum_f32": (_i, [_vp, _vp, _ll, _i, _i, _f, _f, _vp, _vp]),
    "dspn_sum_f32": (_i, [_vp, _ll, _vp, _vp]),
    "dspn_sgd_momentum_f32": (_i, [_vp, _vp, _vp, _ll, _f, _f, _f, _f, _vp]),
    "dspn_sgd_momentum_segments_f32": (_i, [_vp, _vp, _vp, _vp, _i, _ll, _f, _f, _f, _f, _vp]),
})


for _name in ("dspn_conv2d_forward_bn", "dspn_conv2d_dgrad_bn", "dspn_conv2d_wgrad_bn", "dspn_conv2d_wgrad_slabs",
              "dspn_conv2d_input_sum_grad", "dspn_bn_stats", "dspn_bn_apply", "dspn_bn_backward",
              "dspn_bn_backward_from_sums", "dspn_add", "dspn_relu_backward", "dspn_relu_backward_colsum", "dspn_colsum",
              "dspn_nchw_to_nhwc", "dspn_copy_block", "dspn_tap_sum", "dspn_tap_spread", "dspn_maxpool_forward", "dspn_maxpool_forward_bn",
              "dspn_maxpool_backward_argmax", "dspn_maxpool_backward", "dspn_avgpool_forward", "dspn_avgpool_backward",
              "dspn_avgpool2d_forward", "dspn_avgpool2d_backward", "dspn_softmax_output", "dspn_affine_sampler_forward",
              "dspn_affine_sampler_backward_data", "dspn_affine_sampler_backward_theta",
              "dspn_affine_sampler_backward_data_theta"):
    _lib.register({_name + "_bf16": _lib.SIGNATURES[_name + "_f32"]})
_lib.register({
    "dspn_conv2d_weight_prepare_bf16": (_i, [_vp, _vp, _vp, _i, _i, _i, _i, _vp]),
    "dspn_conv2d_weight_prepare_batch_bf16": (_i, [_vp, _i, _ll, _vp]),
    "dspn_copy_block_bf16_f32": _lib.SIGNATURES["dspn_copy_block_f32"],
    "dspn_copy_block_f32_bf16": _lib.SIGNATURES["dspn_copy_block_f32"],
})


class BnMoving(_c.Structure):
    _fields_ = [("moving_mean", _vp), ("moving_var", _vp), ("momentum", _f), ("mode", _i), ("channels", _i)]


BN_TRACK, BN_GLOBAL = 1, 2
_bnmp = _c.POINTER(BnMoving)
_lib.register({
    "dspn_bn_stats_ex_f32": (_i, _lib.SIGNATURES["dspn_bn_stats_f32"][1][:-1] + [_bnmp, _vp]),
    "dspn_bn_stats_ex_bf16": (_i, _lib.SIGNATURES["dspn_bn_stats_f32"][1][:-1] + [_bnmp, _vp]),
    "dspn_bn_stats_from_tiles_ex_f32": (_i, _lib.SIGNATURES["dspn_bn_stats_from_tiles_f32"][1][:-1] + [_bnmp, _vp]),
})


def bn_moving(moving_mean, moving_var, momentum, mode, channels=0):
    return _c.byref(BnMoving(ptr(moving_mean), ptr(moving_var), float(momentum), int(mode), int(channels)))


def L():
    return _lib.lib()


def _f(name, t):
    if t.dtype == torch.bfloat16:
        return getattr(L(), name + "_bf16")
    assert t.dtype == torch.float32, t.dtype
    return getattr(L(), name + "_f32")


def stream():
    return torch.cuda.current_stream().cuda_stream


def ptr(t):
    return 0 if t is None else t.data_ptr()


_ws = {}


_WS_LANE = 0


class workspace_lane:

    def __init__(self, lane):
        self.lane = lane

    def __enter__(self):
        global _WS_LANE
        self.prev, _WS_LANE = _WS_LANE, self.lane

    def __exit__(self, *a):
        global _WS_LANE
        _WS_LANE = self.prev


def workspace(nbytes, device, tag="nn"):
    key = (tag, device, _WS_LANE)
    buf = _ws.get(key)
    if buf is None or buf.numel() < nbytes:
        buf = torch.empty(max(int(nbytes), 1 << 20), dtype=torch.uint8, device=device)
        _ws[key] = buf
    return buf


_scratch = workspace


def _hw(v):
# ... 295 lines not shown
    ph, pw = _hw(pad)
    bx, bsc, bsh, bmu, brs, brelu, bsums = bn_bwd if bn_bwd is not None else (None, None, None, None, None, False, None)
    check(_f("dspn_conv2d_dgrad_bn", dy)(ptr(dy), ptr(wt), ptr(wt_planes), ptr(out), N, H, W, Cin, ldy, R, S, stride, ph, pw,
                                       dil, Ho, Wo, out.shape[3], int(accumulate), ptr(bx), ptr(bsc), ptr(bsh), ptr(bmu),
                                       ptr(brs), int(brelu), ptr(bsums), 0 if bsums is None else bsums.numel() * 4,
                                       ptr(bn_dy_absmax), math | (MATH_DY_PLANES if dy_planes else 0), ptr(dy_absmax),
                                       ptr(w_absmax), ptr(ws), ws.numel(), stream()), "conv2d_dgrad")
    return out


def _wgrad_absmax(x, dy, in_affine, math, x_absmax, dy_absmax):
    if math == 3 and x.dtype == torch.float32:
        return (absmax(x, in_affine) if x_absmax is None else x_absmax, absmax(dy) if dy_absmax is None else dy_absmax)
    return None, None


def conv2d_wgrad(x, dy, w_shape, stride=1, pad=0, dil=1, out=None, accumulate=False, in_affine=None, math=None,
                 x_absmax=None, dy_absmax=None, dy_planes=False, x_planes=False):
    N, H, W, Cin = x.shape
    Cout, R, S, Cw = w_shape
    assert Cw == Cin
    Ho, Wo, ldy = dy.shape[1], dy.shape[2], dy.shape[3]
    if out is None:
        out = empty(Cout, R, S, Cin, device=x.device)
    nbytes = L().dspn_conv2d_wgrad_workspace_bytes(N, Ho, Wo, Cin, Cout, R, S)
    ws = workspace(nbytes, x.device, "wgrad")
    ph, pw = _hw(pad)
    sc, sh, arelu = in_affine if in_affine is not None else (None, None, False)
    assert x.dtype == dy.dtype and out.dtype == torch.float32
    math = _math_code(math)
    assert not x_planes or (x_absmax is not None and in_affine is None)
    x_absmax, dy_absmax = _wgrad_absmax(x, dy, in_affine, math, x_absmax, dy_absmax)
    check(_f("dspn_conv2d_wgrad_bn", x)(ptr(x), ptr(sc), ptr(sh), int(arelu), ptr(dy), ptr(out), N, H, W, Cin, Cout, ldy,
                                       R, S, stride, ph, pw, dil, Ho, Wo, int(accumulate),
                                       math | (MATH_DY_PLANES if dy_planes else 0) | (MATH_X_PLANES if x_planes else 0),
                                       ptr(x_absmax), ptr(dy_absmax), ptr(ws), ws.numel(), stream()), "conv2d_wgrad")
    return out


def tap_sum(z, bias, cout, R, S, pad, out):
    N, H, W, ldz = z.shape
    ph, pw = _hw(pad)
    assert z.dtype == out.dtype
    check(_f("dspn_tap_sum", z)(ptr(z), ptr(bias), ptr(out), N, H, W, cout, out.shape[3], ldz, R, S, ph, pw, stream()),
          "tap_sum")
    return out


def tap_spread(dy, cout, R, S, pad, out):
    N, H, W, ldy = dy.shape
    ph, pw = _hw(pad)
    assert dy.dtype == out.dtype
    check(_f("dspn_tap_spread", dy)(ptr(dy), ptr(out), N, H, W, cout, ldy, out.shape[3], R, S, ph, pw, stream()),
          "tap_spread")
    return out


def conv2d_wgrad_splits(x_shape, dy_shape, w_shape, stride):
    N, H, W, Cin = x_shape
    Cout, R, S, _ = w_shape
    return L().dspn_conv2d_wgrad_splits(N, dy_shape[1], dy_shape[2], Cin, Cout, R, S, stride)


def conv2d_wgrad_slabs(x, dy, w_shape, slabs, stride=1, pad=0, dil=1, in_affine=None, math=None, x_absmax=None,
                       dy_absmax=None, dy_planes=False, x_planes=False):
    N, H, W, Cin = x.shape
    Cout, R, S, Cw = w_shape
    assert Cw == Cin
    ph, pw = _hw(pad)
    sc, sh, arelu = in_affine if in_affine is not None else (None, None, False)
    assert x.dtype == dy.dtype and slabs.dtype == torch.float32
    math = _math_code(math)
    assert not x_planes or (x_absmax is not None and in_affine is None)
    x_absmax, dy_absmax = _wgrad_absmax(x, dy, in_affine, math, x_absmax, dy_absmax)
    check(_f("dspn_conv2d_wgrad_slabs", x)(ptr(x), ptr(sc), ptr(sh), int(arelu), ptr(dy), ptr(slabs), slabs.numel() * 4,
                                          N, H, W, Cin, Cout, dy.shape[3], R, S, stride, ph, pw, dil, dy.shape[1],
                                          dy.shape[2],
                                          math | (MATH_DY_PLANES if dy_planes else 0) | (MATH_X_PLANES if x_planes else 0),
                                          ptr(x_absmax), ptr(dy_absmax), stream()), "conv2d_wgrad_slabs")


def slab_reduce_table(entries, device):
    rows = np.zeros(len(entries), dtype=[("slab", "<u8"), ("dw", "<u8"), ("n4", "<i8"), ("splits", "<i4"),
                                         ("acc", "<i4"), ("begin", "<i8")])
    total = 0
    for i, (slabs, dw, acc) in enumerate(entries):
        assert dw.numel() % 4 == 0 and slabs.numel() == slabs.shape[0] * dw.numel()
        rows[i] = (slabs.data_ptr(), dw.data_ptr(), dw.numel() // 4, slabs.shape[0], int(acc), total)
        total += dw.numel() // 4
    assert rows.dtype.itemsize == 40
    return torch.from_numpy(rows.view(np.uint8).copy()).to(device), len(entries), total


def slab_reduce_batch(table, n, total4):
    check(L().dspn_conv2d_slab_reduce_batch_f32(ptr(table), n, total4, stream()), "slab_reduce_batch")


def conv2d_input_sum_grad(dy, w, x_shape, stride=1, pad=0, dil=1, out=None):
    N, H, W, Cin = x_shape
    Cout, R, S, _ = w.shape
    Ho, Wo, ldy = dy.shape[1], dy.shape[2], dy.shape[3]
    out = empty(Cin, device=dy.device) if out is None else out
    ws = workspace(L().dspn_conv2d_input_sum_grad_workspace_bytes(Ho, Wo, ldy, R, S), dy.device, "sumgrad")
    ph, pw = _hw(pad)
    check(_f("dspn_conv2d_input_sum_grad", dy)(ptr(dy), ptr(w), ptr(out), N, H, W, Cin, Cout, ldy, R, S, stride,
                                             ph, pw, dil, Ho, Wo, ptr(ws), ws.numel(), stream()),
          "conv2d_input_sum_grad")
    return out


def _rows(x):
    return x.numel() // x.shape[-1]


def bn_stats(x, eps, gamma, beta, mean=None, rstd=None, scale=None, shift=None, moving=None):
    C = x.shape[-1]
    rows = _rows(x)
    mean = empty(C, device=x.device) if mean is None else mean
    rstd = empty(C, device=x.device) if rstd is None else rstd
    scale = empty(C, device=x.device) if scale is None else scale
    shift = empty(C, device=x.device) if shift is None else shift
    ws = workspace(L().dspn_bn_workspace_bytes(rows, C), x.device, "bn")
    args = (ptr(x), rows, C, eps, ptr(gamma), ptr(beta), ptr(mean), ptr(rstd), ptr(scale), ptr(shift), ptr(ws), ws.numel())
    if moving is None:
        check(_f("dspn_bn_stats", x)(*args, stream()), "bn_stats")
    else:
        check(_f("dspn_bn_stats_ex", x)(*args, moving, stream()), "bn_stats_ex")
    return mean, rstd, scale, shift


def bn_apply(x, scale, shift, relu=False, out=None, out_absmax=None):
    out = torch.empty_like(x) if out is None else out
    assert out.dtype == x.dtype and (out_absmax is None or out_absmax.numel() == ABSMAX_SLOTS)
    check(_f("dspn_bn_apply", x)(ptr(x), ptr(scale), ptr(shift), ptr(out), _rows(x), x.shape[-1], int(relu),
                                ptr(out_absmax if x.dtype == torch.float32 else None), stream()), "bn_apply")
    return out


def bn_apply_planes(x, scale, shift, y_absmax, relu=False, out=None):
    out = torch.empty_like(x) if out is None else out
    assert x.dtype == out.dtype == torch.float32 and x.shape[-1] % 32 == 0 and y_absmax.numel() == ABSMAX_SLOTS
    check(L().dspn_bn_apply_planes_f32(ptr(x), ptr(scale), ptr(shift), ptr(out), _rows(x), x.shape[-1], int(relu),
                                       ptr(y_absmax), stream()), "bn_apply_planes")
    return out


def absmax_affine_bound(scale, shift, x_absmax, out):
    assert scale.numel() == shift.numel() and x_absmax.numel() == out.numel() == ABSMAX_SLOTS
    check(L().dspn_absmax_affine_bound_f32(ptr(scale), ptr(shift), scale.numel(), ptr(x_absmax), ptr(out), stream()),
          "absmax_affine_bound")
    return out


NO_OUTPUT = type("NoOutput", (), {"__repr__": lambda self: "NO_OUTPUT"})()


def _bn_outputs(x, gamma, dx, dgamma, dbeta):
    C = x.shape[-1]
    dx = None if dx is NO_OUTPUT else (torch.empty_like(x) if dx is None else dx)
    dbeta = None if dbeta is NO_OUTPUT else (empty(C, device=x.device) if dbeta is None else dbeta)
    if dgamma is NO_OUTPUT:
        dgamma = None
    elif gamma is not None and dgamma is None:
        dgamma = empty(C, device=x.device)
    assert dx is None or dx.dtype == x.dtype
    return dx, dgamma, dbeta


def bn_backward(x, scale, shift, dy, mean, rstd, gamma, relu=False, dx=None, dgamma=None, dbeta=None,
                accumulate=False, dx_absmax=None):
    C = x.shape[-1]
    rows = _rows(x)
    dx, dgamma, dbeta = _bn_outputs(x, gamma, dx, dgamma, dbeta)
# ... 1 lines not shown
    assert dy.dtype == x.dtype
    check(_f("dspn_bn_backward", x)(ptr(x), ptr(scale), ptr(shift), ptr(dy), ptr(mean), ptr(rstd), ptr(gamma), ptr(dx),
                                   ptr(dgamma), ptr(dbeta), rows, C, int(relu), int(accumulate), ptr(dx_absmax), ptr(ws),
                                   ws.numel(), stream()), "bn_backward")
    return dx, dgamma, dbeta


def bn_backward_maxpool(x, scale, shift, dy_pool, argmax, k, stride, pad, mean, rstd, gamma, relu=False, dx=None, dgamma=None,
                        dbeta=None, dx_absmax=None):
    N, H, W, C = x.shape
    assert x.dtype == dy_pool.dtype == torch.float32 and argmax.dtype == torch.uint8 and argmax.shape == dy_pool.shape
    dx, dgamma, dbeta = _bn_outputs(x, gamma, dx, dgamma, dbeta)
    ws = workspace(L().dspn_bn_workspace_bytes(N * H * W, C), x.device, "bn")
    check(L().dspn_bn_backward_maxpool_f32(ptr(x), ptr(scale), ptr(shift), ptr(dy_pool), ptr(argmax), N, H, W, C, k, stride, pad,
                                           dy_pool.shape[1], dy_pool.shape[2], ptr(mean), ptr(rstd), ptr(gamma), ptr(dx),
                                           ptr(dgamma), ptr(dbeta), int(relu), ptr(dx_absmax), ptr(ws), ws.numel(), stream()),
          "bn_backward_maxpool")
    return dx, dgamma, dbeta


def bn_backward_from_sums(x, scale, shift, dy, mean, rstd, gamma, sums, tiles, relu=False, dx=None, dgamma=None,
                          dbeta=None, accumulate=False, dx_absmax=None, dy_absmax=None, x_chan_minmax=None, dx_planes=False,
                          dx_absmin=None, phase=0, park=False, workspace=None):
    assert phase in (0, 1, 2) and (not park or phase == 1)
    C = x.shape[-1]
    rows = _rows(x)
    dx, dgamma, dbeta = _bn_outputs(x, gamma, dx, dgamma, dbeta)
    if dx is None:
        assert phase == 0 and not park and not dx_planes, "dx=NO_OUTPUT is a whole call"
        phase = 1
    if workspace is None:
        workspace = _scratch(12 * C + L().dspn_bn_tiles_workspace_bytes(tiles, C), x.device, "bn_from_sums")
    assert dy.dtype == x.dtype
    check(_f("dspn_bn_backward_from_sums", x)(ptr(x), ptr(scale), ptr(shift), ptr(dy), ptr(mean), ptr(rstd), ptr(gamma),
                                             ptr(sums), tiles, ptr(dx), ptr(dgamma), ptr(dbeta), rows, C, int(relu),
                                             int(accumulate), ptr(dx_absmax), ptr(dx_absmin), ptr(dy_absmax), ptr(x_chan_minmax),
                                             int(bool(dx_planes)) | (phase << 1) | (8 if park else 0), ptr(workspace),
                                             workspace.numel(), stream()),
          "bn_backward_from_sums")
    return dx, dgamma, dbeta


def bn_from_sums_workspace(tiles, C, device):
    return torch.empty(12 * C + L().dspn_bn_tiles_workspace_bytes(tiles, C), dtype=torch.uint8, device=device)


def bn_discard_parked(stream_handle):
    return L().dspn_bn_discard_parked(stream_handle)


def add(a, b, out=None):
    out = torch.empty_like(a) if out is None else out
    assert a.dtype == b.dtype == out.dtype
    check(_f("dspn_add", a)(ptr(a), ptr(b), ptr(out), a.numel(), stream()), "add")
    return out


def relu_backward(y, dy, dx=None, accumulate=False):
    dx = torch.empty_like(y) if dx is None else dx
    assert y.dtype == dy.dtype == dx.dtype
    check(_f("dspn_relu_backward", y)(ptr(y), ptr(dy), ptr(dx), y.numel(), int(accumulate), stream()),
          "relu_backward")
    return dx


def relu_backward_colsum(y, dy, C, dx=None, out=None, dx_absmax=None):
    dx = dy if dx is None else dx
    ld = y.shape[-1]
    rows = _rows(y)
    out = empty(C, device=y.device) if out is None else out
    ws = workspace(L().dspn_colsum_workspace_bytes(rows, C), y.device, "colsum")
    assert y.dtype == dy.dtype == dx.dtype
    assert dx_absmax is None or (y.dtype == torch.float32 and dx_absmax.numel() == ABSMAX_SLOTS)
    check(_f("dspn_relu_backward_colsum", y)(ptr(y), ptr(dy), ptr(dx), rows, C, ld, ptr(out), ptr(dx_absmax), ptr(ws), ws.numel(),
                                             stream()), "relu_backward_colsum")
    return dx, out


def fill(t, v):
    check(L().dspn_fill_f32(ptr(t), float(v), t.numel(), stream()), "fill")
    return t


def colsum(a, C, out=None):
    ld = a.shape[-1]
    rows = _rows(a)
    out = empty(C, device=a.device) if out is None else out
    ws = workspace(L().dspn_colsum_workspace_bytes(rows, C), a.device, "colsum")
    check(_f("dspn_colsum", a)(ptr(a), rows, C, ld, ptr(out), ptr(ws), ws.numel(), stream()), "colsum")
    return out


def nchw_to_nhwc(src, Cp=None, out=None):
    N, C, H, W = src.shape
    Cp = (pad4(C) if out is None else out.shape[3]) if Cp is None else Cp
    out = empty(N, H, W, Cp, device=src.device) if out is None else out
    assert src.dtype == torch.float32
    check(_f("dspn_nchw_to_nhwc", out)(ptr(src), ptr(out), N, C, H, W, Cp, stream()), "nchw_to_nhwc")
    return out


def nhwc_to_nchw(src, C=None, out=None):
    N, H, W, Cp = src.shape
    C = Cp if C is None else C
    out = empty(N, C, H, W, device=src.device) if out is None else out
    check(L().dspn_nhwc_to_nchw_f32(ptr(src), ptr(out), N, C, H, W, Cp, stream()), "nhwc_to_nchw")
    return out


def copy_block_table(entries, device):
    rows = np.zeros(len(entries), dtype=[("src", "<u8"), ("dst", "<u8"), ("rps", "<i8"), ("sss", "<i8"), ("dss", "<i8"),
                                         ("C", "<i4"), ("lds", "<i4"), ("soff", "<i4"), ("ldd", "<i4"), ("doff", "<i4"),
                                         ("acc", "<i4"), ("begin", "<i8")])
    assert rows.dtype.itemsize == 72
    total = 0
    for i, (src, dst, samples, rps, C, sss, lds, soff, dss, ldd, doff, acc) in enumerate(entries):
        assert src.dtype == dst.dtype == torch.float32 and samples > 0 and rps > 0 and C > 0
        rows[i] = (src.data_ptr(), dst.data_ptr(), rps, sss, dss, C, lds, soff, ldd, doff, int(bool(acc)), total)
        total += samples * rps * C
    return torch.from_numpy(rows.view(np.uint8).copy()).to(device), len(entries), total


def copy_block_batch(table, n, total):
    check(L().dspn_copy_block_batch_f32(ptr(table), n, total, stream()), "copy_block_batch")


def copy_block(src, dst, samples, rows_per_sample, C, src_sample_stride, lds, soff, dst_sample_stride, ldd,
               doff, accumulate=False):
    if src.dtype == dst.dtype:
        f = _f("dspn_copy_block", src)
    elif src.dtype == torch.bfloat16:
        f = L().dspn_copy_block_bf16_f32
    else:
        f = L().dspn_copy_block_f32_bf16
    check(f(ptr(src), ptr(dst), samples, rows_per_sample, C, src_sample_stride, lds,
                                  soff, dst_sample_stride, ldd, doff, int(accumulate), stream()), "copy_block")
    return dst


def transpose_bnc(src, out=None):
    B, N, C = src.shape
    out = empty(B, C, N, device=src.device) if out is None else out
    check(L().dspn_transpose_bnc_f32(ptr(src), ptr(out), B, N, C, stream()), "transpose_bnc")
    return out


def maxpool_forward(x, k, stride, pad, out=None, argmax=None, in_affine=None, out_absmax=None):
    N, H, W, C = x.shape
    if out is None:
        out = empty(N, conv_out_size(H, k, stride, pad), conv_out_size(W, k, stride, pad), C, device=x.device, dtype=x.dtype)
    Ho, Wo = out.shape[1], out.shape[2]
    assert argmax is None or (argmax.dtype == torch.uint8 and argmax.shape == out.shape)
    assert out.dtype == x.dtype
    if in_affine is not None:
        sc, sh, relu = in_affine
        check(_f("dspn_maxpool_forward_bn", x)(ptr(x), ptr(sc), ptr(sh), int(bool(relu)), ptr(out), ptr(argmax), N, H, W, C, k,
                                             stride, pad, Ho, Wo, ptr(out_absmax if x.dtype == torch.float32 else None), stream()),
              "maxpool_forward_bn")
        return out
    check(_f("dspn_maxpool_forward", x)(ptr(x), ptr(out), ptr(argmax), N, H, W, C, k, stride, pad, Ho, Wo, stream()),
          "maxpool_forward")
    return out


def maxpool_backward_argmax(argmax, dy, x_shape, k, stride, pad, dx=None):
    N, H, W, C = x_shape
    dx = empty(N, H, W, C, device=dy.device, dtype=dy.dtype) if dx is None else dx
    assert dx.dtype == dy.dtype
    check(_f("dspn_maxpool_backward_argmax", dy)(ptr(argmax), ptr(dy), ptr(dx), N, H, W, C, k, stride, pad,
                                               dy.shape[1], dy.shape[2], stream()), "maxpool_backward_argmax")
    return dx
# ... 237 lines not shown
```

### dspnet_amd/symbol/common.py

```python
import numpy as np

from .. import engine as E
from .. import functional as fn
from .. import operator as op


def conv_act_layer(g, from_layer, name, num_filter, kernel=1, pad=0, stride=1):
    return g.add(E.Conv(g, from_layer, "{}_conv".format(name), num_filter, kernel, stride, pad,
                        no_bias=False, relu=True, init="maxdim")).out


def multi_layer_feature(g, internals, from_layers, num_filters, strides, pads, min_filter=128):
    assert len(from_layers) > 0
    assert isinstance(from_layers[0], str) and len(from_layers[0].strip()) > 0
    assert len(from_layers) == len(num_filters) == len(strides) == len(pads)
    layers = []
    for k, (from_layer, num_filter, s, p) in enumerate(zip(from_layers, num_filters, strides, pads)):
        if from_layer.strip():
            t = internals[from_layer.strip() + "_output"]
            t.ssd_name = from_layer.strip()
            layers.append(t)
        else:
            assert len(layers) > 0 and num_filter > 0
            num_1x1 = max(min_filter, num_filter // 2)
            c1 = conv_act_layer(g, layers[-1], "multi_feat_%d_conv_1x1" % k, num_1x1, 1, 0, 1)
            c3 = conv_act_layer(g, c1, "multi_feat_%d_conv_3x3" % k, num_filter, 3, p, s)
            c3.ssd_name = "multi_feat_%d_conv_3x3_relu" % k
            layers.append(c3)
    return layers


class HeadPack(E.Node):

    def __init__(self, g, maps, widths, name):
        self.maps, self.widths = maps, widths
        B = maps[0].shape[0]
        self.sizes = [t.shape[1] * t.shape[2] * c for t, c in zip(maps, widths)]
        self.offsets = np.cumsum([0] + self.sizes).tolist()
        self.total = self.offsets[-1]
        import torch
        self.out = g.tensor((B, self.total), name, dtype=torch.float32)
        self._tables = {}

    def _batched(self, key, entries):
        import torch
        if self.out.data.device.type != "cuda" or any(e[0].dtype != torch.float32 or e[1].dtype != torch.float32 for e in entries):
            return False
        key = (key,) + tuple((e[0].data_ptr(), e[1].data_ptr(), bool(e[-1])) for e in entries)
        tab = self._tables.get(key)
        if tab is None:
            tab = self._tables[key] = fn.copy_block_table(entries, self.out.data.device)
        fn.copy_block_batch(*tab)
        return True

    def forward(self):
        B = self.out.shape[0]
        entries = [(t.data, self.out.data, B, t.shape[1] * t.shape[2], c, t.shape[1] * t.shape[2] * t.shape[3], t.shape[3], 0,
                    self.total, c, off, False) for t, c, off in zip(self.maps, self.widths, self.offsets)]
        if not self._batched("f", entries):
            for e in entries:
                fn.copy_block(*e[:-1])

    def backward(self):
        if not self.out._gw:
            return
        B = self.out.shape[0]
        entries = []
        for t, c, off in zip(self.maps, self.widths, self.offsets):
            hw = t.shape[1] * t.shape[2]
            dx, acc = t.grad_target()
            entries.append((self.out.grad, dx, B, hw, c, self.total, c, off, hw * t.shape[3], t.shape[3], 0, acc))
        if not self._batched("b", entries):
            for e in entries:
                fn.copy_block(*e[:-1], accumulate=e[-1])


def multitask_layer(g, from_layers, num_classes, sizes, ratios, normalization=-1, clip=False, steps=()):
    assert len(from_layers) > 0, "from_layers must not be empty list"
    assert num_classes > 0, "num_classes {} must be larger than 0".format(num_classes)
    assert len(ratios) == len(from_layers), "ratios and from_layers must have same length"
    assert len(sizes) == len(from_layers), "sizes and from_layers must have same length"
    if not isinstance(normalization, (list, tuple)):
        normalization = [normalization] * len(from_layers)
    assert all(n <= 0 for n in normalization), "L2Normalization heads are not part of the DSPNet presets that build"
    num_classes += 1
    loc_maps, cls_maps, loc_w, cls_w, anchors = [], [], [], [], []
    for k, from_layer in enumerate(from_layers):
        from_name = from_layer.ssd_name
        size, ratio = sizes[k], ratios[k]
        num_anchors = len(size) - 1 + len(ratio)
        big = from_layer.shape[0] * from_layer.shape[1] * from_layer.shape[2] >= 4096
        loc = g.add(E.Conv(g, from_layer, "{}_loc_pred_conv".format(from_name), num_anchors * 5, 3, 1, 1,
                           no_bias=False, init="maxdim", tap_expand=big)).out
        cls = g.add(E.Conv(g, from_layer, "{}_cls_pred_conv".format(from_name), num_anchors * num_classes, 3,
                           1, 1, no_bias=False, init="maxdim", tap_expand=big)).out
        for t in (loc, cls):
            t.producer.b.lr_mult = 2.0
        loc_maps.append(loc); loc_w.append(num_anchors * 5)
        cls_maps.append(cls); cls_w.append(num_anchors * num_classes)
        step = (steps[k], steps[k]) if steps else (-1.0, -1.0)
        anchors.append(op.MultiBoxPrior((from_layer.shape[1], from_layer.shape[2]), sizes=size, ratios=ratio,
                                        clip=clip, steps=step))
    loc_preds = g.add(HeadPack(g, loc_maps, loc_w, "multibox_loc_pred")).out
    cls_flat = g.add(HeadPack(g, cls_maps, cls_w, "multibox_cls_flat")).out
    import torch
    anchor_boxes = torch.cat(anchors, dim=1).contiguous()
    return loc_preds, cls_flat, anchor_boxes
```

### dspnet_amd/train/solver.py

```python
from .. import functional as fn


def plan_buckets(params, owner_index, total, bucket_elems, frozen=None):
    if frozen:
        return _plan_buckets_frozen(params, owner_index, bucket_elems, set(frozen))
    buckets, lo, first = [], 0, None
    for name, offset, size in params:
        idx = owner_index[name]
        first = idx if first is None else min(first, idx)
        end = offset + size
        if end - lo >= bucket_elems:
            buckets.append((lo, end, first))
            lo, first = end, None
    if lo < total:
        buckets.append((lo, total, first if first is not None else 0))
    buckets.sort(key=lambda b: -b[2])
    return buckets


def _plan_buckets_frozen(params, owner_index, bucket_elems, frozen):
    buckets, lo, first, end = [], None, None, None
    for name, offset, size in params:
        if name in frozen:
            if lo is not None:
# ... 68 lines not shown
                self._issue_ev.append(ev)
            self.works.append(dist.all_reduce(self.arena[lo:hi], group=self.pg, async_op=True))

    def finish(self):
        assert not self.pending, "backward ended before every bucket was released"
        timed = self.measure_exposed and self.arena.is_cuda
        if timed:
            import torch
            e0, e1 = torch.cuda.Event(enable_timing=True), torch.cuda.Event(enable_timing=True)
            e0.record()
        done_ev = []
        for w in self.works:
            w.wait()
            if timed and len(done_ev) < len(self._issue_ev):
                ev = torch.cuda.Event(enable_timing=True)
                ev.record()
                done_ev.append(ev)
        if timed:
            e1.record()
            self.exposed_events.append((e0, e1))
            if len(done_ev) == len(self._issue_ev):
                self.bucket_events.append(list(zip(self._issue_ev, done_ev)))

    def exposed_ms(self):
        if not self.exposed_events:
            return None
        t = sum(a.elapsed_time(b) for a, b in self.exposed_events) / len(self.exposed_events)
        self.exposed_events = []
        return t

    def bucket_latency_ms(self):
        if not self.bucket_events:
            return None
        n = len(self.bucket_events[0])
        out = [sum(step[b][0].elapsed_time(step[b][1]) for step in self.bucket_events) / len(self.bucket_events) for b in range(n)]
        self.bucket_events = []
        return out


class MultiTaskSolver:
    def __init__(self, net, learning_rate=0.0005, momentum=0.9, wd=0.0005, process_group=None,
                 world_size=1, bucket_mb=16.0, force_reducer=False, high_priority=True, track_bn_stats=True,
                 aux_params=None, optimizer_rules="multi_solver", rescale_grad=None):
        if optimizer_rules not in OPTIMIZER_RULES:
            raise ValueError("optimizer_rules must be one of %s, got %r" % (OPTIMIZER_RULES, optimizer_rules))
        self.optimizer_rules, self.rescale_grad = optimizer_rules, rescale_grad
        self.net, self.g = net, net.g
        self.track_bn_stats = bool(track_bn_stats)
        if aux_params:
            net.g.set_aux(aux_params, allow_missing=True)
        self.stream = None
        if high_priority and net.g.device.type == "cuda":
            import torch
            from ..engine import shared_stream
            self.stream = shared_stream(net.g.device, "step", -1)
        self.lr, self.momentum, self.wd = learning_rate, momentum, wd
        self.world_size, self.pg = world_size, process_group
        self.batch_size = net.data.shape[0]
        self._graph, self._graph_hyper = None, None
        self._ran_eager = False
        self._rerecord = False
        self._replays, self.graph_rerecorded = 0, 0
        g = self.g
        owner = {}
        for idx, n in enumerate(g.nodes):
            for p in n.wiring.params:
                owner.setdefault(p.name, idx)
        params = [(p.name, p.offset, (p.size + 3) // 4 * 4) for p in g.param_order]
        fixed = {p.name for p in g.param_order if p.fixed}
        self.buckets = plan_buckets(params, owner, g.arena.numel(), int(bucket_mb * (1 << 20) / 4), frozen=fixed or None)
        self.sgd_rows = self.sgd_table = None
        if fixed or optimizer_rules == "module":
            self.sgd_rows = sgd_segments([(p.offset, (p.size + 3) // 4 * 4)
                                          + rule_multipliers(p.name, optimizer_rules, p.lr_mult, p.wd_mult)
                                          for p in g.param_order if not p.fixed])
            if self.sgd_rows and g.device.type == "cuda":
                self.sgd_table = fn.sgd_segment_table(self.sgd_rows, g.arena.numel(), g.device)
        self.reducer = (GradBucketReducer(g.grad_arena, self.buckets, process_group)
                        if (world_size > 1 or force_reducer) else None)
        g.wgrad_side_allowed = self.reducer is None
        self.bucket_convs = []
        for lo, hi, first in self.buckets:
            self.bucket_convs.append((first, [n for n in g.nodes if getattr(n, "slabs", None) is not None
                                              and lo <= n.w.offset < hi]))
        self.bucket_side = side_buckets(self.buckets, params, owner,
                                        g.side_bwd["side"] if g.side_bwd is not None else ())

    def set_batch(self, data, label_det, label_seg):
        self.net.data.data.copy_(data)
        if self.net.label_det is not None:
            self.net.label_det.data.copy_(label_det)
        if self.net.label_seg is not None:
            self.net.label_seg.data.copy_(label_seg)

    def forward(self):
        self.g.forward()

    def _train_forward(self):
        g = self.g
        g.bn_track = self.track_bn_stats
        try:
            g.forward()
        finally:
            g.bn_track = False

    def backward(self):
        g = self.g
        g.begin_backward()
        if self.reducer is not None:
            self.reducer.begin()
        if self.reducer is None:
            pending = list(range(len(self.bucket_convs)))
            for idx in range(len(g.nodes) - 1, -1, -1):
                g.backward_node(idx)
                while pending and self.bucket_convs[pending[0]][0] >= idx and not g.side_backward_busy(idx):
                    b = pending.pop(0)
                    g.flush_slabs(("bucket", b), self.bucket_convs[b][1], beside=True)
            g.join_side_backward()
            for b in pending:
                g.flush_slabs(("bucket", b), self.bucket_convs[b][1])
            return

        def before_release(b):
            if self.bucket_side[b]:
                g.join_side_backward()
            g.flush_slabs(("bucket", b), self.bucket_convs[b][1])

        for idx in range(len(g.nodes) - 1, -1, -1):
            g.backward_node(idx)
            self.reducer.node_done(idx, before_release)
        g.join_side_backward()
        self.reducer.finish()

    def rescale(self):
        if self.rescale_grad is not None:
            return float(self.rescale_grad)
        if self.optimizer_rules == "module":
            return 1.0 / self.world_size
        return 1.0 / (self.batch_size * self.world_size)

    def update(self):
        g = self.g
        if self.sgd_rows is None:
            fn.sgd_momentum(g.arena, g.grad_arena, g.mom_arena, self.lr, self.momentum, self.wd, self.rescale())
        elif not self.sgd_rows:
            return
        elif self.sgd_table is None:
            raise RuntimeError("MultiTaskSolver.update: the segmented update runs on a GPU graph only (this one is on %s)"
                               % g.device)
        else:
            fn.sgd_momentum_segments(g.arena, g.grad_arena, g.mom_arena, self.sgd_table, self.lr, self.momentum, self.wd,
                                     self.rescale())

    def _on_step_stream(self, body):
        if self.stream is None:
            return body()
        import torch
        cur = torch.cuda.current_stream(self.g.device)
        if cur == self.stream:
            return body()
        self.stream.wait_stream(cur)
        with torch.cuda.stream(self.stream):
            body()
        cur.wait_stream(self.stream)

    def step(self):
        self._on_step_stream(self._step)
# ... 148 lines not shown
```

### include/dspn_nn.h

```cpp
#ifndef DSPN_NN_H_
#define DSPN_NN_H_

#include <stddef.h>

#ifdef __cplusplus
extern "C" {
#endif


size_t dspn_conv2d_split_workspace_bytes(long long out_pixels, int Cout);
#define DSPN_MATH_FP32 0
#define DSPN_MATH_BF16 1
#define DSPN_MATH_F32_BF16X3 2
#define DSPN_MATH_F32_F16X2 3
#define DSPN_MATH_UNSCALED_OK 0x100
#define DSPN_MATH_DY_PLANES 0x200
#define DSPN_MATH_X_PLANES 0x400

int dspn_conv2d_forward_f32(const float *x, const float *w, const float *bias, const float *residual, float *y,
                            int N, int H, int W, int Cin, int Cout, int R, int S,
                            int stride, int pad_h, int pad_w, int dil, int Ho, int Wo,
                            long long y_batch_stride, int y_ldc, int relu, int accumulate,
                            void *workspace, size_t workspace_bytes, void *stream);

// ... 74 lines not shown
                                long long y_batch_stride, int y_ldc, int relu, int accumulate,
                                float *out_stats, size_t out_stats_bytes, float *out_minmax_unused, int math,
                                const float *absmax_unused_a, const float *absmax_unused_b,
                                void *workspace, size_t workspace_bytes, void *stream);
int dspn_conv2d_dgrad_bn_bf16(const dspn_bf16 *dy, const dspn_bf16 *wt, const void *wt_planes_unused, dspn_bf16 *dx, int N, int H, int W, int Cin,
                              int ldy, int R, int S, int stride, int pad_h, int pad_w, int dil, int Ho, int Wo,
                              int dx_ldc, int accumulate, const dspn_bf16 *bn_x, const float *bn_scale,
                              const float *bn_shift, const float *bn_mean, const float *bn_rstd, int bn_relu,
                              float *bn_sums, size_t bn_sums_bytes, float *bn_dy_absmax_unused, int math,
                              const float *absmax_unused_a, const float *absmax_unused_b, void *workspace,
                              size_t workspace_bytes, void *stream);
int dspn_conv2d_wgrad_bn_bf16(const dspn_bf16 *x, const float *in_scale, const float *in_shift, int in_relu,
                              const dspn_bf16 *dy, float *dw, int N, int H, int W, int Cin, int Cout, int ldy,
                              int R, int S, int stride, int pad_h, int pad_w, int dil, int Ho, int Wo,
                              int accumulate, int math, const float *absmax_unused_a, const float *absmax_unused_b,
                              void *workspace, size_t workspace_bytes, void *stream);
int dspn_conv2d_wgrad_slabs_bf16(const dspn_bf16 *x, const float *in_scale, const float *in_shift, int in_relu,
                                 const dspn_bf16 *dy, float *slabs, size_t slabs_bytes, int N, int H, int W, int Cin,
                                 int Cout, int ldy, int R, int S, int stride, int pad_h, int pad_w, int dil, int Ho,
                                 int Wo, int math, const float *absmax_unused_a, const float *absmax_unused_b, void *stream);
int dspn_conv2d_input_sum_grad_bf16(const dspn_bf16 *dy, const float *w, float *out, int N, int H, int W,
                                    int Cin, int Cout, int ldy, int R, int S, int stride, int pad_h, int pad_w, int dil,
                                    int Ho, int Wo, void *workspace, size_t workspace_bytes, void *stream);
int dspn_conv2d_weight_prepare_bf16(const float *w, dspn_bf16 *wh, dspn_bf16 *wt, int Cout, int taps, int Cin,
                                    int Cout_pad, void *stream);
int dspn_conv2d_weight_prepare_batch_bf16(const void *table, int n, long long total_tiles, void *stream);


size_t dspn_bn_workspace_bytes(long long rows, int C);

int dspn_bn_stats_f32(const float *x, long long rows, int C, float eps, const float *gamma,
                      const float *beta, float *mean, float *rstd, float *scale, float *shift,
                      void *workspace, size_t workspace_bytes, void *stream);

int dspn_bn_stats_from_tiles_f32(const float *tile_stats, int tiles, int tile_rows, long long rows, int C, float eps,
                                 const float *gamma, const float *beta, float *mean, float *rstd, float *scale,
                                 float *shift, const float *tile_minmax, int relu, float *out_absmax, float *out_absmin,
                                 float *out_chan_minmax, void *workspace, size_t workspace_bytes, void *stream);
size_t dspn_bn_tiles_workspace_bytes(int tiles, int C);

#define DSPN_BN_TRACK 1
#define DSPN_BN_GLOBAL 2
typedef struct dspn_bn_moving {
  float *moving_mean;
  float *moving_var;
  float momentum;
  int mode;
  int channels;
} dspn_bn_moving;
int dspn_bn_stats_ex_f32(const float *x, long long rows, int C, float eps, const float *gamma,
                         const float *beta, float *mean, float *rstd, float *scale, float *shift,
                         void *workspace, size_t workspace_bytes, const dspn_bn_moving *moving, void *stream);
int dspn_bn_stats_from_tiles_ex_f32(const float *tile_stats, int tiles, int tile_rows, long long rows, int C, float eps,
                                    const float *gamma, const float *beta, float *mean, float *rstd, float *scale,
                                    float *shift, const float *tile_minmax, int relu, float *out_absmax, float *out_absmin,
                                    float *out_chan_minmax, void *workspace, size_t workspace_bytes,
                                    const dspn_bn_moving *moving, void *stream);

int dspn_bn_apply_f32(const float *x, const float *scale, const float *shift, float *y, long long rows,
                      int C, int relu, float *out_absmax, void *stream);
int dspn_bn_apply_planes_f32(const float *x, const float *scale, const float *shift, void *y_planes, long long rows, int C,
                             int relu, const float *y_absmax, void *stream);

int dspn_bn_backward_f32(const float *x, const float *scale, const float *shift, const float *dy,
                         const float *mean, const float *rstd, const float *gamma, float *dx,
                         float *dgamma, float *dbeta, long long rows, int C, int relu, int accumulate,
                         float *dx_absmax, void *workspace, size_t workspace_bytes, void *stream);
int dspn_bn_backward_from_sums_f32(const float *x, const float *scale, const float *shift, const float *dy,
                                   const float *mean, const float *rstd, const float *gamma, const float *tile_sums,
                                   int tiles, float *dx, float *dgamma, float *dbeta, long long rows, int C, int relu,
                                   int accumulate, float *dx_absmax, float *dx_absmin, const float *dy_absmax, const float *x_chan_minmax,
                                   int dx_planes, void *workspace, size_t workspace_bytes, void *stream);
int dspn_bn_discard_parked(void *stream);

int dspn_add_f32(const float *a, const float *b, float *out, long long n, void *stream);
int dspn_relu_backward_f32(const float *y, const float *dy, float *dx, long long n, int accumulate, void *stream);
int dspn_relu_backward_colsum_f32(const float *y, const float *dy, float *dx, long long rows, int C, int ld,
                                  float *out, float *dx_absmax ,
                                  void *workspace, size_t workspace_bytes, void *stream);
int dspn_fill_f32(float *p, float v, long long n, void *stream);
size_t dspn_colsum_workspace_bytes(long long rows, int C);
int dspn_colsum_f32(const float *a, long long rows, int C, int ld, float *out,
                    void *workspace, size_t workspace_bytes, void *stream);
int dspn_nchw_to_nhwc_f32(const float *src, float *dst, int N, int C, int H, int W, int Cp, void *stream);
int dspn_nhwc_to_nchw_f32(const float *src, float *dst, int N, int C, int H, int W, int Cp, void *stream);
int dspn_copy_block_f32(const float *src, float *dst, int samples, long long rows_per_sample, int C,
                        long long src_sample_stride, int lds, int soff,
                        long long dst_sample_stride, int ldd, int doff, int accumulate, void *stream);
int dspn_copy_block_batch_f32(const void *table, int n, long long total, void *stream);
int dspn_transpose_bnc_f32(const float *src, float *dst, int B, int N, int C, void *stream);

int dspn_tap_sum_f32(const float *z, const float *bias, float *y, int N, int H, int W, int Cout, int ldy,
                     int ldz, int R, int S, int pad_h, int pad_w, void *stream);
int dspn_tap_spread_f32(const float *dy, float *dz, int N, int H, int W, int Cout, int ldy, int ldz, int R,
                        int S, int pad_h, int pad_w, void *stream);

int dspn_maxpool_forward_f32(const float *x, float *y, unsigned char *argmax, int N, int H, int W, int C, int k,
                             int stride, int pad, int Ho, int Wo, void *stream);
int dspn_maxpool_forward_bn_f32(const float *x, const float *in_scale, const float *in_shift, int in_relu, float *y,
                                unsigned char *argmax, int N, int H, int W, int C, int k, int stride, int pad, int Ho, int Wo,
                                float *out_absmax, void *stream);
int dspn_bn_backward_maxpool_f32(const float *x, const float *scale, const float *shift, const float *dy_pool,
                                 const unsigned char *argmax, int N, int H, int W, int C, int k, int stride, int pad, int Ho,
                                 int Wo, const float *mean, const float *rstd, const float *gamma, float *dx, float *dgamma,
                                 float *dbeta, int relu, float *dx_absmax, void *workspace, size_t workspace_bytes, void *stream);
int dspn_maxpool_backward_argmax_f32(const unsigned char *argmax, const float *dy, float *dx, int N, int H,
                                     int W, int C, int k, int stride, int pad, int Ho, int Wo, void *stream);
int dspn_maxpool_backward_f32(const float *x, const float *y, const float *dy, float *dx, int N, int H,
                              int W, int C, int k, int stride, int pad, int Ho, int Wo, void *stream);
int dspn_avgpool_forward_f32(const float *x, float *y, int N, int H, int W, int C, int k, int Ho, int Wo, void *stream);
int dspn_avgpool_backward_f32(const float *dy, float *dx, int N, int H, int W, int C, int k, int Ho, int Wo,
                              int accumulate, void *stream);

int dspn_avgpool2d_forward_f32(const float *x, float *y, int N, int H, int W, int C, int k, int stride, int pad,
                               int Ho, int Wo, void *stream);
int dspn_avgpool2d_backward_f32(const float *dy, float *dx, int N, int H, int W, int C, int k, int stride, int pad,
                                int Ho, int Wo, int accumulate, void *stream);

int dspn_bilinear_forward_f32(const float *x, float *y, int N, int Hin, int Win, int C, int Ho, int Wo,
                              int ldo, int coff, void *stream);
int dspn_bilinear_forward_acc_f32(const float *x, float *y, int N, int Hin, int Win, int C, int Ho, int Wo,
                                  int ldo, int coff, void *stream);
int dspn_bilinear_backward_f32(const float *dy, float *dx, int N, int Hin, int Win, int C, int Ho, int Wo,
                               int ldo, int coff, void *stream);
size_t dspn_bilinear_backward_workspace_bytes(int N, int Win, int C, int Ho);
int dspn_bilinear_backward_ws_f32(const float *dy, float *dx, int N, int Hin, int Win, int C, int Ho, int Wo,
                                  int ldo, int coff, void *workspace, size_t workspace_bytes, void *stream);

#define DSPN_SAMPLER_MAX_SOURCES 8
int dspn_affine_sampler_forward_f32(const float *const *x, const int *Hin, const int *Win, const int *C, const int *coff,
                                    int nsrc, const float *theta, float *y, int N, int Ho, int Wo, int ldo, void *stream);
int dspn_affine_sampler_backward_data_f32(const float *dy, const float *theta, float *dx, int N, int Hin, int Win, int C,
                                          int Ho, int Wo, int ldo, int coff, int accumulate, void *stream);
size_t dspn_affine_sampler_theta_workspace_bytes(int N, int Ho, int Wo);
int dspn_affine_sampler_backward_theta_f32(const float *const *x, const int *Hin, const int *Win, const int *C,
                                           const int *coff, int nsrc, const float *theta, const float *dy, int N, int Ho,
                                           int Wo, int ldo, float *dtheta, int accumulate, void *workspace,
                                           size_t workspace_bytes, void *stream);
int dspn_affine_sampler_backward_data_theta_f32(const float *dy, const float *theta, const float *x, float *dx, int N, int Hin,
                                                int Win, int C, int Ho, int Wo, int ldo, int coff, int accumulate,
                                                double *theta_partial, size_t theta_partial_bytes, float *dx_absmax,
                                                void *workspace, size_t workspace_bytes, void *stream);
long long dspn_affine_sampler_theta_rows(int N, int Hin, int Win, int Ho);
size_t dspn_affine_sampler_backward_workspace_bytes(int N, int Hin, int Win, int C, int Ho);
size_t dspn_affine_sampler_theta_reduce_workspace_bytes(long long rows);
int dspn_affine_sampler_theta_reduce(const double *theta_partial, long long rows, float *dtheta, int accumulate, void *workspace,
                                     size_t workspace_bytes, void *stream);

int dspn_seg_counts_f32(const float *scores, const float *label, long long rows, int C, int ld,
                        unsigned long long *counts, void *stream);

int dspn_seg_upsample_argmax_f32(const float *prob, unsigned char *out, int N, int Hin, int Win, int C, int ld,
                                 int Ho, int Wo, void *stream);

int dspn_softmax_output_f32(const float *logits, const float *label, float *prob, float *grad,
                            long long rows, int C, int ld, float ignore_label, float grad_scale,
                            const float *valid_count, void *stream);
int dspn_count_f32(const float *a, long long n, int mode, float ref, float *out, void *stream);
int dspn_smooth_l1_forward_f32(const float *pred, const float *target, const float *mask, float *loss,
                               long long n, void *stream);
int dspn_smooth_l1_backward_f32(const float *pred, const float *target, const float *mask, float *grad,
                                long long n, float grad_scale, const float *valid_count, void *stream);
int dspn_cross_entropy_sum_f32(const float *prob, const float *label, long long rows, int C, int ld,
                               float ignore_label, float eps, float *out2, void *stream);
int dspn_sum_f32(const float *a, long long n, float *out, void *stream);

int dspn_sgd_momentum_f32(float *w, const float *grad, float *mom, long long n, float lr, float momentum,
                          float wd, float rescale, void *stream);

#define DSPN_SGD_MAX_SEGMENTS 8192
typedef struct dspn_sgd_segment {
  long long offset;
  long long length;
  float lr_mult;
  float wd_mult;
} dspn_sgd_segment;
int dspn_sgd_momentum_segments_f32(float *w, const float *grad, float *mom, const dspn_sgd_segment *segments, int nseg,
                                   long long total4, float lr, float momentum, float wd, float rescale, void *stream);

int dspn_bn_stats_bf16(const dspn_bf16 *x, long long rows, int C, float eps, const float *gamma,
                      const float *beta, float *mean, float *rstd, float *scale, float *shift,
                      void *workspace, size_t workspace_bytes, void *stream);
int dspn_bn_stats_ex_bf16(const dspn_bf16 *x, long long rows, int C, float eps, const float *gamma,
                          const float *beta, float *mean, float *rstd, float *scale, float *shift,
                          void *workspace, size_t workspace_bytes, const dspn_bn_moving *moving, void *stream);
int dspn_bn_apply_bf16(const dspn_bf16 *x, const float *scale, const float *shift, dspn_bf16 *y, long long rows,
                      int C, int relu, float *out_absmax , void *stream);
int dspn_bn_backward_bf16(const dspn_bf16 *x, const float *scale, const float *shift, const dspn_bf16 *dy,
                         const float *mean, const float *rstd, const float *gamma, dspn_bf16 *dx,
                         float *dgamma, float *dbeta, long long rows, int C, int relu, int accumulate,
                         float *dx_absmax_unused, void *workspace, size_t workspace_bytes, void *stream);
int dspn_bn_backward_from_sums_bf16(const dspn_bf16 *x, const float *scale, const float *shift, const dspn_bf16 *dy,
                                   const float *mean, const float *rstd, const float *gamma, const float *tile_sums,
                                   int tiles, dspn_bf16 *dx, float *dgamma, float *dbeta, long long rows, int C, int relu,
                                   int accumulate, float *dx_absmax_unused, float *dx_absmin_unused, const float *dy_absmax_unused,
                                   const float *x_chan_minmax_unused, int dx_planes , void *workspace,
                                   size_t workspace_bytes, void *stream);
int dspn_add_bf16(const dspn_bf16 *a, const dspn_bf16 *b, dspn_bf16 *out, long long n, void *stream);
int dspn_relu_backward_bf16(const dspn_bf16 *y, const dspn_bf16 *dy, dspn_bf16 *dx, long long n, int accumulate, void *stream);
int dspn_relu_backward_colsum_bf16(const dspn_bf16 *y, const dspn_bf16 *dy, dspn_bf16 *dx, long long rows, int C, int ld,
                                  float *out, float *dx_absmax_unused , void *workspace, size_t workspace_bytes,
                                  void *stream);
int dspn_colsum_bf16(const dspn_bf16 *a, long long rows, int C, int ld, float *out,
                    void *workspace, size_t workspace_bytes, void *stream);
int dspn_nchw_to_nhwc_bf16(const float *src, dspn_bf16 *dst, int N, int C, int H, int W, int Cp, void *stream);
int dspn_copy_block_bf16(const dspn_bf16 *src, dspn_bf16 *dst, int samples, long long rows_per_sample, int C,
                        long long src_sample_stride, int lds, int soff,
                        long long dst_sample_stride, int ldd, int doff, int accumulate, void *stream);
int dspn_tap_sum_bf16(const dspn_bf16 *z, const float *bias, dspn_bf16 *y, int N, int H, int W, int Cout, int ldy,
                     int ldz, int R, int S, int pad_h, int pad_w, void *stream);
int dspn_tap_spread_bf16(const dspn_bf16 *dy, dspn_bf16 *dz, int N, int H, int W, int Cout, int ldy, int ldz, int R,
                        int S, int pad_h, int pad_w, void *stream);
int dspn_maxpool_forward_bf16(const dspn_bf16 *x, dspn_bf16 *y, unsigned char *argmax, int N, int H, int W, int C, int k,
                             int stride, int pad, int Ho, int Wo, void *stream);
int dspn_maxpool_forward_bn_bf16(const dspn_bf16 *x, const float *in_scale, const float *in_shift, int in_relu, dspn_bf16 *y,
                                 unsigned char *argmax, int N, int H, int W, int C, int k, int stride, int pad, int Ho, int Wo,
                                 float *out_absmax_unused, void *stream);
int dspn_maxpool_backward_argmax_bf16(const unsigned char *argmax, const dspn_bf16 *dy, dspn_bf16 *dx, int N, int H,
                                     int W, int C, int k, int stride, int pad, int Ho, int Wo, void *stream);
int dspn_maxpool_backward_bf16(const dspn_bf16 *x, const dspn_bf16 *y, const dspn_bf16 *dy, dspn_bf16 *dx, int N, int H,
                              int W, int C, int k, int stride, int pad, int Ho, int Wo, void *stream);
int dspn_avgpool_forward_bf16(const dspn_bf16 *x, dspn_bf16 *y, int N, int H, int W, int C, int k, int Ho, int Wo, void *stream);
int dspn_avgpool_backward_bf16(const dspn_bf16 *dy, dspn_bf16 *dx, int N, int H, int W, int C, int k, int Ho, int Wo,
                              int accumulate, void *stream);
int dspn_avgpool2d_forward_bf16(const dspn_bf16 *x, dspn_bf16 *y, int N, int H, int W, int C, int k, int stride, int pad,
                               int Ho, int Wo, void *stream);
int dspn_avgpool2d_backward_bf16(const dspn_bf16 *dy, dspn_bf16 *dx, int N, int H, int W, int C, int k, int stride, int pad,
                                int Ho, int Wo, int accumulate, void *stream);
int dspn_softmax_output_bf16(const dspn_bf16 *logits, const float *label, float *prob, dspn_bf16 *grad,
                            long long rows, int C, int ld, float ignore_label, float grad_scale,
                            const float *valid_count, void *stream);
int dspn_affine_sampler_backward_data_bf16(const dspn_bf16 *dy, const float *theta, dspn_bf16 *dx, int N, int Hin, int Win, int C,
                                          int Ho, int Wo, int ldo, int coff, int accumulate, void *stream);
int dspn_affine_sampler_backward_data_theta_bf16(const dspn_bf16 *dy, const float *theta, const dspn_bf16 *x, dspn_bf16 *dx, int N,
                                                 int Hin, int Win, int C, int Ho, int Wo, int ldo, int coff, int accumulate,
                                                 double *theta_partial, size_t theta_partial_bytes, float *dx_absmax ,
                                                 void *workspace , size_t workspace_bytes, void *stream);
int dspn_affine_sampler_forward_bf16(const dspn_bf16 *const *x, const int *Hin, const int *Win, const int *C, const int *coff,
                                    int nsrc, const float *theta, dspn_bf16 *y, int N, int Ho, int Wo, int ldo, void *stream);
int dspn_affine_sampler_backward_theta_bf16(const dspn_bf16 *const *x, const int *Hin, const int *Win, const int *C,
                                           const int *coff, int nsrc, const float *theta, const dspn_bf16 *dy, int N, int Ho,
                                           int Wo, int ldo, float *dtheta, int accumulate, void *workspace,
                                           size_t workspace_bytes, void *stream);
int dspn_copy_block_bf16_f32(const dspn_bf16 *src, float *dst, int samples, long long rows_per_sample, int C,
                             long long src_sample_stride, int lds, int soff, long long dst_sample_stride,
                             int ldd, int doff, int accumulate, void *stream);
int dspn_copy_block_f32_bf16(const float *src, dspn_bf16 *dst, int samples, long long rows_per_sample, int C,
                             long long src_sample_stride, int lds, int soff, long long dst_sample_stride,
                             int ldd, int doff, int accumulate, void *stream);

#ifdef __cplusplus
}
#endif
#endif
```

Baseline: 958.3 images/s.

## Merge SSD loc and cls prediction convs into one paired convolution per feature map

Detection heads on backbone feature maps now run as a single ConvPair whose output channels are the concatenation of the loc and cls predictions. Forward, dgrad and wgrad each launch once per map instead of twice, and the input feature map is read once. Per-head parameters are kept, which adds a copy of the merged weights every forward step, a pitched slab reduce that scatters weight gradients back to each head, and a split column-sum for the biases. HeadPack now slices the packed output by start channel.

```diff
diff --git a/dspnet_amd/csrc/conv.hip b/dspnet_amd/csrc/conv.hip
--- a/dspnet_amd/csrc/conv.hip
+++ b/dspnet_amd/csrc/conv.hip
@@ -1333,7 +1333,7 @@
   }
 }
 
-struct SlabDesc { const float4 *slab; float4 *dw; long long n4; int splits, accumulate; long long begin; };
+struct SlabDesc { const float4 *slab; float4 *dw; long long n4; int splits, accumulate; long long begin; long long pitch4; };
 __global__ void slab_reduce_batch_kernel(const SlabDesc *__restrict__ d, int n, long long total) {
   for (long long i = blockIdx.x * (long long)blockDim.x + threadIdx.x; i < total;
        i += (long long)gridDim.x * blockDim.x) {
@@ -1349,12 +1349,12 @@
     for (; k + 16 <= e.splits; k += 16) {
       float4 v[16];
 #pragma unroll
-      for (int u = 0; u < 16; ++u) v[u] = e.slab[(long long)(k + u) * e.n4 + j];
+      for (int u = 0; u < 16; ++u) v[u] = e.slab[(long long)(k + u) * e.pitch4 + j];
 #pragma unroll
       for (int u = 0; u < 16; ++u) { s.x += v[u].x; s.y += v[u].y; s.z += v[u].z; s.w += v[u].w; }
     }
     for (; k < e.splits; ++k) {
-      const float4 v = e.slab[(long long)k * e.n4 + j];
+      const float4 v = e.slab[(long long)k * e.pitch4 + j];
       s.x += v.x; s.y += v.y; s.z += v.z; s.w += v.w;
     }
     if (e.accumulate) { const float4 v = e.dw[j]; s.x += v.x; s.y += v.y; s.z += v.z; s.w += v.w; }
@@ -2291,7 +2291,7 @@
 #ifndef DSPN_HALF
 int dspn_conv2d_slab_reduce_batch_f32(const void *table, int n, long long total4, void *stream) {
   DSPN_REQUIRE(table && n > 0 && total4 > 0, "slab_reduce_batch: bad argument");
-  static_assert(sizeof(SlabDesc) == 40, "table row layout: 2 pointers, int64, 2 ints, int64");
+  static_assert(sizeof(SlabDesc) == 48, "table row layout: 2 pointers, int64, 2 ints, 2 int64");
   const int blocks = (int)std::min<long long>((total4 + 255) / 256, 16384);
   dspn::ProfScope prof(1, (hipStream_t)stream);
   hipLaunchKernelGGL(slab_reduce_batch_kernel, dim3(blocks), dim3(256), 0, (hipStream_t)stream,
diff --git a/dspnet_amd/csrc/nn.hip b/dspnet_amd/csrc/nn.hip
--- a/dspnet_amd/csrc/nn.hip
+++ b/dspnet_amd/csrc/nn.hip
@@ -821,7 +821,8 @@
       if (c4 * 4 + e < C) p[c4 * 4 + e] = v[e];
   }
 }
-__global__ __launch_bounds__(1024) void colsum_final_kernel(const float *partial, int nslabs, int C, float *out) {
+__global__ __launch_bounds__(1024) void colsum_final_kernel(const float *partial, int nslabs, int C, float *out,
+                                                            float *out2 = nullptr, int C1 = 0) {
   __shared__ double sm[64][17];
   const int cl = threadIdx.x & 15, sl = threadIdx.x >> 4;
   const int c = blockIdx.x * 16 + cl;
@@ -834,7 +835,8 @@
   __syncthreads();
   if (sl == 0 && c < C) {
     for (int k = 1; k < 64; ++k) s += sm[k][cl];
-    out[c] = (float)s;
+    if (out2 && c >= C1) out2[c - C1] = (float)s;
+    else out[c] = (float)s;
   }
 }
 
@@ -1962,6 +1964,19 @@
   return dspn::check_launch("colsum");
 }
 
+int DSPN_FN(dspn_colsum_pair)(const st_t *a, long long rows, int C, int ld, float *out, int C1, float *out2, void *workspace,
+                         size_t workspace_bytes, void *stream) {
+  DSPN_REQUIRE(a && out && out2 && workspace && rows > 0 && C1 > 0 && C > C1 && ld >= C, "colsum_pair: bad argument");
+  const int sr = colsum_slab_rows(rows);
+  const int ns = (int)((rows + sr - 1) / sr);
+  if (workspace_bytes < sizeof(float) * (size_t)ns * C)
+    return dspn::fail(DSPN_ERR_WORKSPACE_, "colsum_pair: workspace too small");
+  float *partial = static_cast<float *>(workspace);
+  hipLaunchKernelGGL(colsum_partial_kernel, dim3(ns), dim3(kT), 0, S_(stream), CA1Ptr(a), rows, C, ld, partial, sr);
+  hipLaunchKernelGGL(colsum_final_kernel, dim3((C + 15) / 16), dim3(1024), 0, S_(stream), partial, ns, C, out, out2, C1);
+  return dspn::check_launch("colsum_pair");
+}
+
 int DSPN_FN(dspn_nchw_to_nhwc)(const float *src, st_t *dst, int N, int C, int H, int W, int Cp, void *stream) {
   DSPN_REQUIRE(src && dst && N > 0 && C > 0 && H > 0 && W > 0 && Cp >= C, "nchw_to_nhwc: bad argument");
   const long long HW = (long long)H * W, total = HW * N;
diff --git a/dspnet_amd/engine.py b/dspnet_amd/engine.py
--- a/dspnet_amd/engine.py
+++ b/dspnet_amd/engine.py
@@ -185,6 +185,7 @@
         self.side_plan = None
         self.slab_tables = {}
         self.wt_table = None
+        self.pair_table = None
         self.wt_batched = False
         self.arena = self.grad_arena = self.mom_arena = None
         self.half_operands = False
@@ -378,6 +379,10 @@
         for p in self.param_order:
             p.data = self.arena[p.offset:p.offset + p.size].view(p.shape)
             p.grad = self.grad_arena[p.offset:p.offset + p.size].view(p.shape)
+        if self.device.type == "cuda":
+            rows = [r for n in self.nodes if isinstance(n, ConvPair) for r in n.merge_rows()]
+            if rows:
+                self.pair_table = fn.copy_block_table(rows, self.device)
         if self._wt_pairs_nodes and self.device.type == "cuda":
             for n in self._wt_pairs_nodes:
                 if n.wt is None:
@@ -455,7 +460,7 @@
     def _slab_table(self, key, convs):
         if key not in self.slab_tables:
             nodes = [n for n in convs if isinstance(n, Conv) and n.slabs is not None]
-            table = fn.slab_reduce_table([(n.slabs, n.w.grad, False) for n in nodes], self.device) if nodes else None
+            table = fn.slab_reduce_table([e for n in nodes for e in n.slab_entries()], self.device) if nodes else None
             self.slab_tables[key] = (nodes, table)
         return self.slab_tables[key]
 
@@ -481,6 +486,8 @@
 
     def forward(self):
         self.wt_batched = False
+        if self.pair_table is not None:
+            fn.copy_block_batch(*self.pair_table)
         if self.half_operands:
             fn.weight_transpose_batch(*self.wt_table)
             self.wt_batched = True
@@ -984,11 +991,7 @@
         self.input_sum_grad = input_sum_grad
         cin_meta = cin_logical if cin_logical is not None else (x.channels or Cin)
         cin_logical = Cin if cin_logical is None else cin_logical
-        self.w = g.param(name + "_weight", (num_filter, kh, kw, Cin), conv_weight_init(init, cin_logical))
-        self.b = None if no_bias else g.param(name + "_bias", (num_filter,), init_zeros)
-        self.w.logical, self.w.kind = (num_filter, cin_meta, kh, kw), "conv"
-        if self.b is not None:
-            self.b.logical = (num_filter,)
+        self.w, self.b = self._make_params(g, name, (num_filter, kh, kw, Cin), init, cin_logical, cin_meta, no_bias)
         Ho, Wo = fn.conv_out_size(H, kh, stride, ph, dilate), fn.conv_out_size(W, kw, stride, pw, dilate)
         ldc = fn.padc(num_filter) if cout_phys is None else cout_phys
         self.out = g.tensor((N, Ho, Wo, ldc), out_name or (name + "_out"))
@@ -1036,6 +1039,24 @@
         self.flops_fwd = 2.0 * cin_logical * num_filter * kh * kw * Ho * Wo * N
         self.flops_bwd = self.flops_fwd * (2 if x.requires_grad else 1)
 
+    def _make_params(self, g, name, shape, init, cin_logical, cin_meta, no_bias):
+        num_filter, kh, kw, _ = shape
+        w = g.param(name + "_weight", shape, conv_weight_init(init, cin_logical))
+        b = None if no_bias else g.param(name + "_bias", (num_filter,), init_zeros)
+        w.logical, w.kind = (num_filter, cin_meta, kh, kw), "conv"
+        if b is not None:
+            b.logical = (num_filter,)
+        return w, b
+
+    def slab_entries(self):
+        return [(self.slabs, self.w.grad, False)]
+
+    def grad_offsets(self):
+        return [self.w.offset]
+
+    def _bias_gradient(self, dy):
+        fn.colsum(dy, self.cout, out=self.b.grad)
+
     def alloc_slabs(self):
         if self.w.fixed:
             return
@@ -1158,7 +1179,7 @@
         if self.residual is not None and self.residual.requires_grad:
             self.residual.give_grad(dy)
         if self.b is not None and not self.relu and not self.b.fixed:
-            fn.colsum(dy, self.cout, out=self.b.grad)
+            self._bias_gradient(dy)
         xa, dya, wa = self._magnitudes("x"), self._magnitudes("dy"), self._magnitudes("w")
         if dya is not None and self.am_dy not in self._g._am_done:
             fn.absmax(dy, out=dya)
@@ -1259,6 +1280,83 @@
         fn.conv2d_dgrad(dy, self.wt, self.x.shape, self.stride, self.pad, self.dil, out=dx, accumulate=acc,
                         bn_bwd=bn_bwd, wt_planes=self.wtp, math=self.math, dy_absmax=dya, w_absmax=wa,
                         bn_dy_absmax=bn_dya, dy_planes=planes, wt_shape=self.wt_shape)
+
+
+class Merged:
+
+    def __init__(self, parts, device):
+        self.parts = parts
+        self.name = "+".join(p.name for p in parts)
+        self.shape = (sum(p.shape[0] for p in parts),) + tuple(parts[0].shape[1:])
+        self.fixed, self.lr_mult = False, 1.0
+        self.data = fn.zeros(*self.shape, device=device)
+        self.direct_grad = None
+        if len(self.shape) == 4:
+            self.logical, self.kind = (sum(p.logical[0] for p in parts),) + tuple(parts[0].logical[1:]), "conv"
+        else:
+            self.logical, self.kind = (self.shape[0],), "vec"
+
+    @property
+    def offset(self):
+        return self.parts[0].offset
+
+    @property
+    def grad(self):
+        return self.direct_grad if self.direct_grad is not None else torch.cat([p.grad for p in self.parts], 0)
+
+    def rows(self):
+        out, r = [], 0
+        for p in self.parts:
+            out.append((r, p.shape[0]))
+            r += p.shape[0]
+        return out
+
+
+class ConvPair(Conv):
+
+    def __init__(self, g, x, name, num_loc, num_cls, kernel=3, stride=1, pad=1, tap_expand=False):
+        self.widths = (num_loc, num_cls)
+        Conv.__init__(self, g, x, name, num_loc + num_cls, kernel, stride, pad, no_bias=False, init="maxdim",
+                      cout_phys=(num_loc + num_cls + 31) // 32 * 32, tap_expand=tap_expand, out_name=name + "_pair_out")
+
+    def _make_params(self, g, name, shape, init, cin_logical, cin_meta, no_bias):
+        _, kh, kw, cin = shape
+        self.heads = []
+        for kind, n in zip(("loc", "cls"), self.widths):
+            self.heads += list(Conv._make_params(self, g, "%s_%s_pred_conv" % (name, kind), (n, kh, kw, cin), init, cin_logical,
+                                                 cin_meta, no_bias))
+        assert not any(p.fixed for p in self.heads), "a pair with a frozen head is built as two Conv (multitask_layer)"
+        return Merged(self.heads[0::2], g.device), Merged(self.heads[1::2], g.device)
+
+    def merge_rows(self):
+        rows = []
+        for m in (self.w, self.b):
+            ld = int(np.prod(m.shape[1:])) if len(m.shape) > 1 else 1
+            for p, (r0, nr) in zip(m.parts, m.rows()):
+                rows.append((p.data, m.data[r0:r0 + nr], 1, nr, ld, 0, ld, 0, 0, ld, 0, False))
+        return rows
+
+    def alloc_slabs(self):
+        Conv.alloc_slabs(self)
+        if self.slabs is None:
+            self.w.direct_grad = fn.zeros(*self.w.shape, device=self._g.device)
+
+    def slab_entries(self):
+        per_row = int(np.prod(self.w.shape[1:]))
+        return [(self.slabs, p.grad, False, r0 * per_row) for p, (r0, _) in zip(self.w.parts, self.w.rows())]
+
+    def grad_offsets(self):
+        return [p.offset for p in self.w.parts]
+
+    def _bias_gradient(self, dy):
+        fn.colsum(dy, self.cout, out=self.b.parts[0].grad, split=(self.widths[0], self.b.parts[1].grad))
+
+    def _weight_gradient(self, dy, planes, xa, dya):
+        Conv._weight_gradient(self, dy, planes, xa, dya)
+        if self.slabs is None:
+            ld = int(np.prod(self.w.shape[1:]))
+            for p, (r0, nr) in zip(self.w.parts, self.w.rows()):
+                fn.copy_block(self.w.direct_grad[r0:r0 + nr], p.grad, 1, nr, ld, 0, ld, 0, 0, ld, 0)
 
 
 class BilinearConcatConv(Node):
diff --git a/dspnet_amd/functional.py b/dspnet_amd/functional.py
--- a/dspnet_amd/functional.py
+++ b/dspnet_amd/functional.py
@@ -66,6 +66,7 @@
     "dspn_relu_backward_colsum_f32": (_i, [_vp, _vp, _vp, _ll, _i, _i, _vp, _vp, _vp, _sz, _vp]),
     "dspn_colsum_workspace_bytes": (_sz, [_ll, _i]),
     "dspn_colsum_f32": (_i, [_vp, _ll, _i, _i, _vp, _vp, _sz, _vp]),
+    "dspn_colsum_pair_f32": (_i, [_vp, _ll, _i, _i, _vp, _i, _vp, _vp, _sz, _vp]),
     "dspn_nchw_to_nhwc_f32": (_i, [_vp, _vp, _i, _i, _i, _i, _i, _vp]),
     "dspn_nhwc_to_nchw_f32": (_i, [_vp, _vp, _i, _i, _i, _i, _i, _vp]),
     "dspn_copy_block_f32": (_i, [_vp, _vp, _i, _ll, _i, _ll, _i, _i, _ll, _i, _i, _i, _vp]),
@@ -114,7 +115,7 @@
 
 for _name in ("dspn_conv2d_forward_bn", "dspn_conv2d_dgrad_bn", "dspn_conv2d_wgrad_bn", "dspn_conv2d_wgrad_slabs",
               "dspn_conv2d_input_sum_grad", "dspn_bn_stats", "dspn_bn_apply", "dspn_bn_backward",
-              "dspn_bn_backward_from_sums", "dspn_add", "dspn_relu_backward", "dspn_relu_backward_colsum", "dspn_colsum",
+              "dspn_bn_backward_from_sums", "dspn_add", "dspn_relu_backward", "dspn_relu_backward_colsum", "dspn_colsum", "dspn_colsum_pair",
               "dspn_nchw_to_nhwc", "dspn_copy_block", "dspn_tap_sum", "dspn_tap_spread", "dspn_maxpool_forward", "dspn_maxpool_forward_bn",
               "dspn_maxpool_backward_argmax", "dspn_maxpool_backward", "dspn_avgpool_forward", "dspn_avgpool_backward",
               "dspn_avgpool2d_forward", "dspn_avgpool2d_backward", "dspn_softmax_output", "dspn_affine_sampler_forward",
@@ -576,13 +577,17 @@
 
 def slab_reduce_table(entries, device):
     rows = np.zeros(len(entries), dtype=[("slab", "<u8"), ("dw", "<u8"), ("n4", "<i8"), ("splits", "<i4"),
-                                         ("acc", "<i4"), ("begin", "<i8")])
+                                         ("acc", "<i4"), ("begin", "<i8"), ("pitch4", "<i8")])
     total = 0
-    for i, (slabs, dw, acc) in enumerate(entries):
-        assert dw.numel() % 4 == 0 and slabs.numel() == slabs.shape[0] * dw.numel()
-        rows[i] = (slabs.data_ptr(), dw.data_ptr(), dw.numel() // 4, slabs.shape[0], int(acc), total)
+    for i, e in enumerate(entries):
+        slabs, dw, acc = e[:3]
+        first = e[3] if len(e) > 3 else 0
+        pitch = slabs.numel() // slabs.shape[0]
+        assert dw.numel() % 4 == 0 and first % 4 == 0 and pitch % 4 == 0 and 0 <= first and first + dw.numel() <= pitch
+        assert len(e) > 3 or pitch == dw.numel()
+        rows[i] = (slabs.data_ptr() + 4 * first, dw.data_ptr(), dw.numel() // 4, slabs.shape[0], int(acc), total, pitch // 4)
         total += dw.numel() // 4
-    assert rows.dtype.itemsize == 40
+    assert rows.dtype.itemsize == 48
     return torch.from_numpy(rows.view(np.uint8).copy()).to(device), len(entries), total
 
 
@@ -750,11 +755,17 @@
     return t
 
 
-def colsum(a, C, out=None):
+def colsum(a, C, out=None, split=None):
     ld = a.shape[-1]
     rows = _rows(a)
     out = empty(C, device=a.device) if out is None else out
     ws = workspace(L().dspn_colsum_workspace_bytes(rows, C), a.device, "colsum")
+    if split is not None:
+        C1, out2 = split
+        assert 0 < C1 < C and out.numel() >= C1 and out2.numel() >= C - C1
+        check(_f("dspn_colsum_pair", a)(ptr(a), rows, C, ld, ptr(out), C1, ptr(out2), ptr(ws), ws.numel(), stream()),
+              "colsum_pair")
+        return out
     check(_f("dspn_colsum", a)(ptr(a), rows, C, ld, ptr(out), ptr(ws), ws.numel(), stream()), "colsum")
     return out
 
diff --git a/dspnet_amd/symbol/common.py b/dspnet_amd/symbol/common.py
--- a/dspnet_amd/symbol/common.py
+++ b/dspnet_amd/symbol/common.py
@@ -32,8 +32,9 @@
 
 class HeadPack(E.Node):
 
-    def __init__(self, g, maps, widths, name):
+    def __init__(self, g, maps, widths, name, starts=None):
         self.maps, self.widths = maps, widths
+        self.starts = list(starts) if starts is not None else [0] * len(maps)
         B = maps[0].shape[0]
         self.sizes = [t.shape[1] * t.shape[2] * c for t, c in zip(maps, widths)]
         self.offsets = np.cumsum([0] + self.sizes).tolist()
@@ -55,8 +56,8 @@
 
     def forward(self):
         B = self.out.shape[0]
-        entries = [(t.data, self.out.data, B, t.shape[1] * t.shape[2], c, t.shape[1] * t.shape[2] * t.shape[3], t.shape[3], 0,
-                    self.total, c, off, False) for t, c, off in zip(self.maps, self.widths, self.offsets)]
+        entries = [(t.data, self.out.data, B, t.shape[1] * t.shape[2], c, t.shape[1] * t.shape[2] * t.shape[3], t.shape[3], s0,
+                    self.total, c, off, False) for t, c, off, s0 in zip(self.maps, self.widths, self.offsets, self.starts)]
         if not self._batched("f", entries):
             for e in entries:
                 fn.copy_block(*e[:-1])
@@ -66,16 +67,22 @@
             return
         B = self.out.shape[0]
         entries = []
-        for t, c, off in zip(self.maps, self.widths, self.offsets):
+        for t, c, off, s0 in zip(self.maps, self.widths, self.offsets, self.starts):
             hw = t.shape[1] * t.shape[2]
             dx, acc = t.grad_target()
-            entries.append((self.out.grad, dx, B, hw, c, self.total, c, off, hw * t.shape[3], t.shape[3], 0, acc))
+            if isinstance(t.producer, E.ConvPair):
+                acc = False
+            entries.append((self.out.grad, dx, B, hw, c, self.total, c, off, hw * t.shape[3], t.shape[3], s0, acc))
         if not self._batched("b", entries):
             for e in entries:
                 fn.copy_block(*e[:-1], accumulate=e[-1])
 
 
-def multitask_layer(g, from_layers, num_classes, sizes, ratios, normalization=-1, clip=False, steps=()):
+PAIR_HEADS = True
+
+
+def multitask_layer(g, from_layers, num_classes, sizes, ratios, normalization=-1, clip=False, steps=(), pair_heads=None):
+    pair_heads = PAIR_HEADS if pair_heads is None else pair_heads
     assert len(from_layers) > 0, "from_layers must not be empty list"
     assert num_classes > 0, "num_classes {} must be larger than 0".format(num_classes)
     assert len(ratios) == len(from_layers), "ratios and from_layers must have same length"
@@ -85,24 +92,36 @@
     assert all(n <= 0 for n in normalization), "L2Normalization heads are not part of the DSPNet presets that build"
     num_classes += 1
     loc_maps, cls_maps, loc_w, cls_w, anchors = [], [], [], [], []
+    loc_s, cls_s = [], []
     for k, from_layer in enumerate(from_layers):
         from_name = from_layer.ssd_name
         size, ratio = sizes[k], ratios[k]
         num_anchors = len(size) - 1 + len(ratio)
         big = from_layer.shape[0] * from_layer.shape[1] * from_layer.shape[2] >= 4096
-        loc = g.add(E.Conv(g, from_layer, "{}_loc_pred_conv".format(from_name), num_anchors * 5, 3, 1, 1,
-                           no_bias=False, init="maxdim", tap_expand=big)).out
-        cls = g.add(E.Conv(g, from_layer, "{}_cls_pred_conv".format(from_name), num_anchors * num_classes, 3,
-                           1, 1, no_bias=False, init="maxdim", tap_expand=big)).out
-        for t in (loc, cls):
-            t.producer.b.lr_mult = 2.0
+        names = ["{}_{}_pred_conv_{}".format(from_name, k, p) for k in ("loc", "cls") for p in ("weight", "bias")]
+        on_backbone = not from_name.startswith("multi_feat_")
+        if pair_heads and on_backbone and not (g.freezing and any(g.is_fixed(n) for n in names)):
+            pair = g.add(E.ConvPair(g, from_layer, from_name, num_anchors * 5, num_anchors * num_classes, tap_expand=big))
+            loc = cls = pair.out
+            biases = pair.heads[1::2]
+            loc_s.append(0); cls_s.append(num_anchors * 5)
+        else:
+            loc = g.add(E.Conv(g, from_layer, "{}_loc_pred_conv".format(from_name), num_anchors * 5, 3, 1, 1,
+                               no_bias=False, init="maxdim", tap_expand=big)).out
+            cls = g.add(E.Conv(g, from_layer, "{}_cls_pred_conv".format(from_name), num_anchors * num_classes, 3,
+                               1, 1, no_bias=False, init="maxdim", tap_expand=big)).out
+            biases = [loc.producer.b, cls.producer.b]
+            loc_s.append(0); cls_s.append(0)
+        for b in biases:
+            b.lr_mult = 2.0
         loc_maps.append(loc); loc_w.append(num_anchors * 5)
         cls_maps.append(cls); cls_w.append(num_anchors * num_classes)
         step = (steps[k], steps[k]) if steps else (-1.0, -1.0)
         anchors.append(op.MultiBoxPrior((from_layer.shape[1], from_layer.shape[2]), sizes=size, ratios=ratio,
                                         clip=clip, steps=step))
-    loc_preds = g.add(HeadPack(g, loc_maps, loc_w, "multibox_loc_pred")).out
-    cls_flat = g.add(HeadPack(g, cls_maps, cls_w, "multibox_cls_flat")).out
+    sliced = any(cls_s)
+    loc_preds = g.add(HeadPack(g, loc_maps, loc_w, "multibox_loc_pred", loc_s if sliced else None)).out
+    cls_flat = g.add(HeadPack(g, cls_maps, cls_w, "multibox_cls_flat", cls_s if sliced else None)).out
     import torch
     anchor_boxes = torch.cat(anchors, dim=1).contiguous()
     return loc_preds, cls_flat, anchor_boxes
diff --git a/dspnet_amd/train/solver.py b/dspnet_amd/train/solver.py
--- a/dspnet_amd/train/solver.py
+++ b/dspnet_amd/train/solver.py
@@ -174,7 +174,7 @@
         self.bucket_convs = []
         for lo, hi, first in self.buckets:
             self.bucket_convs.append((first, [n for n in g.nodes if getattr(n, "slabs", None) is not None
-                                              and lo <= n.w.offset < hi]))
+                                              and any(lo <= o < hi for o in n.grad_offsets())]))
         self.bucket_side = side_buckets(self.buckets, params, owner,
                                         g.side_bwd["side"] if g.side_bwd is not None else ())
 
diff --git a/include/dspn_nn.h b/include/dspn_nn.h
--- a/include/dspn_nn.h
+++ b/include/dspn_nn.h
@@ -180,6 +180,8 @@
 size_t dspn_colsum_workspace_bytes(long long rows, int C);
 int dspn_colsum_f32(const float *a, long long rows, int C, int ld, float *out,
                     void *workspace, size_t workspace_bytes, void *stream);
+int dspn_colsum_pair_f32(const float *a, long long rows, int C, int ld, float *out, int C1, float *out2,
+                         void *workspace, size_t workspace_bytes, void *stream);
 int dspn_nchw_to_nhwc_f32(const float *src, float *dst, int N, int C, int H, int W, int Cp, void *stream);
 int dspn_nhwc_to_nchw_f32(const float *src, float *dst, int N, int C, int H, int W, int Cp, void *stream);
 int dspn_copy_block_f32(const float *src, float *dst, int samples, long long rows_per_sample, int C,
@@ -301,6 +303,8 @@
                                   void *stream);
 int dspn_colsum_bf16(const dspn_bf16 *a, long long rows, int C, int ld, float *out,
                     void *workspace, size_t workspace_bytes, void *stream);
+int dspn_colsum_pair_bf16(const dspn_bf16 *a, long long rows, int C, int ld, float *out, int C1, float *out2,
+                          void *workspace, size_t workspace_bytes, void *stream);
 int dspn_nchw_to_nhwc_bf16(const float *src, dspn_bf16 *dst, int N, int C, int H, int W, int Cp, void *stream);
 int dspn_copy_block_bf16(const dspn_bf16 *src, dspn_bf16 *dst, int samples, long long rows_per_sample, int C,
                         long long src_sample_stride, int lds, int soff,
```

Result: no change. 966.4 images/s (median of 6 runs) (+0.8%).
